# ChantalMP/RaDialog

Measured on AMD Instinct MI355X. Metric: reports_per_sec (448px CXR encode + 160-tok prefill + 256-tok greedy decode), higher is better.
Workload: dtype bf16; 1 GPU; configs[1]: per-GPU batch 1 BioViL-T(ResNet-50)+Q-Former encode 448px, Vicuna-7B prefill T=160, 256-token greedy decode (LoRA r=8 un-merged, hipGraph ; per_gpu_batch=1, global_batch=1, prompt_len=160, parallelism=dp1

## Files before the change

### include/rdx_dec_hooks.h

```cpp
#ifndef RDX_DEC_HOOKS_H
#define RDX_DEC_HOOKS_H
#include "rdx.h"
#ifdef __cplusplus
extern "C" {
#endif

int rdx_xstat16_test(rdx_ctx* ctx, const void* X, const void* norm_w, float eps, const float* W, int M, int N, int epi, int n_valid, void* out,
                     int ldo, int out_packed, int32_t* argmax_host);

int rdx_xrow16_test(rdx_ctx* ctx, const void* X, int x_packed, const float* W, const void* resid, int M, int N, int K, void* out, int ldo);

int rdx_xstat_blk_test(rdx_ctx* ctx, const void* X, const void* norm_w, float eps, const float* W, const void* resid, int M, int N, int epi,
                       int n_valid, void* out, int ldo, int out_packed, void* xp_out, int32_t* argmax_host);

int rdx_xsplit_blk_test(rdx_ctx* ctx, const void* X, const float* W, void* x_resid, const void* norm_w, float eps, int M, int N, float* slab_out,
                        void* xn_out);

int rdx_xstat_blk8_test(rdx_ctx* ctx, const void* X, const void* norm_w, float eps, const float* W, int M, int N, int epi, int n_valid, void* out,
                        int ldo, int out_packed, void* x8_out, float* xscale_out, int32_t* argmax_host);

int rdx_xsplit_blk8_test(rdx_ctx* ctx, const void* X, const float* W, void* x_resid, const void* norm_w, float eps, int M, int N, int K,
                         float* slab_out, void* x8_out, float* xscale_out);

int rdx_rmsnorm_test(rdx_ctx* ctx, void* x, const void* norm_w, float eps, int rows, int H, int layout, int mtiles, const float* slab, int groups, void* out,
                     long long out_bytes, float* xscale, int xscale_n);

int rdx_select_test(rdx_ctx* ctx, void* logits_inout, int B, int vocab, const int32_t* hist, const int32_t* hist_len, const int32_t* n_generated, int ld,
                    const rdx_logits_rules* rules, int eos_id, int32_t* tokens_out);

int rdx_decode_attn_test(rdx_ctx* ctx, int heads, int B, int max_len, int k_perm, int lora_r, float lora_scale, const void* qkv, const void* lbq, const void* lbv,
                         const void* cur_rope, const void* cos_t, const void* sin_t, int max_pos, const int32_t* pos, const int32_t* slot,
                         const uint8_t* key_mask, void* kcache, void* vcache, void* out, long long out_bytes, int out_packed, int out_mt);

int rdx_rope_kv_test(rdx_ctx* ctx, int heads, int B, int T, int max_len, int k_perm, int lora_r, float lora_scale, const void* qkv, const void* lbq,
                     const void* lbv, const void* cos_t, const void* sin_t, int max_pos, const int32_t* pos_ids, int slot0, void* kcache, void* vcache,
                     void* qout);

int rdx_sample_test(rdx_ctx* ctx, void* logits_inout, int B, int vocab, const int32_t* hist, const int32_t* hist_len, const int32_t* n_generated, int ld,
                    const rdx_logits_rules* rules, int eos_id, const rdx_sampling* sampling, int32_t* tokens_out);
int rdx_sample_u24_host(uint64_t seed, uint32_t row, uint32_t draw, uint32_t* out);

#ifdef __cplusplus
}
#endif
#endif
```

### radialog_amd/_lib.py

```python
from __future__ import annotations

import ctypes as C
import os

import torch

HERE = os.path.dirname(os.path.abspath(__file__))
LIB_PATH = os.environ.get("RDX_LIB_PATH") or os.path.join(HERE, "librdx.so")
HOOKS_PATH = os.environ.get("RDX_HOOKS_PATH") or os.path.join(HERE, "librdx_hooks.so")

RDX_DTYPE_F16, RDX_DTYPE_BF16 = 0, 1
RDX_W_GEMM, RDX_W_TENSOR, RDX_W_F32, RDX_W_GEMM_FP8 = 0, 1, 2, 3
RDX_SRC_F32, RDX_SRC_F16, RDX_SRC_BF16 = 0, 1, 2


class RdxLibraryError(RuntimeError):
    pass


class RdxError(RuntimeError):
    pass


class RdxLogitsRules(C.Structure):
# ... 66 lines not shown
    "rdx_quant_test": (C.c_int, [_P, _P, C.c_int, C.c_int, C.c_int, C.c_int, _P, C.c_float, _P, _P]),
    "rdx_gemv_trace": (C.c_int, [_P, C.c_int, C.c_int, _P, C.c_int]),
    "rdx_gemm_test": (C.c_int, [_P, _P, _P, _P, _P, _P, C.c_int, C.c_int, C.c_int, C.c_int, _P, C.c_float, C.c_int]),
    "rdx_kernel_bench": (C.c_int, [_P, C.c_int, C.c_int, C.c_int, C.c_int, C.c_int, C.c_int, C.c_int, C.c_int, C.POINTER(C.c_float), _P, C.c_int]),
    "rdx_conv_test": (C.c_int, [_P, _P, _P, _P, _P, _P, C.c_int, C.c_int, C.c_int, C.c_int, C.c_int, C.c_int, C.c_int, C.c_int, C.c_int, C.POINTER(C.c_float)]),
    "rdx_l2_bench": (C.c_int, [_P, C.c_int, C.c_longlong, C.c_int, C.c_int, C.c_int, C.POINTER(C.c_float)]),
    "rdx_logits_test": (C.c_int, [_P, _P, _P, C.c_int, C.c_int, C.c_int, C.c_int, _P, _P, C.c_int]),
}

TRACE_CHAIN = 7
TRACE_ATTN_OPROJ = 8

ENC_HOOK_SYMBOLS = {
    "rdx_stem_test": (C.c_int, [_P, _P, _P, _P, _P, C.c_int, C.c_int, C.c_int, C.c_int]),
    "rdx_norm_test": (C.c_int, [_P, C.c_int, _P, _P, _P, _P, _P, _P, C.c_int, C.c_int, C.c_longlong, C.c_longlong, C.c_int, C.c_int, C.c_float]),
    "rdx_attn_test": (C.c_int, [_P, _P, _P, _P, _P, _P, C.c_int, C.c_int, C.c_int, C.c_int, C.c_int, C.c_int, _P, C.c_longlong, C.c_int, C.c_int]),
}

_F = C.c_float
DEC_HOOK_SYMBOLS = {
    "rdx_xstat16_test": (C.c_int, [_P, _P, _P, _F, _P, C.c_int, C.c_int, C.c_int, C.c_int, _P, C.c_int, C.c_int, _P]),
    "rdx_xrow16_test": (C.c_int, [_P, _P, C.c_int, _P, _P, C.c_int, C.c_int, C.c_int, _P, C.c_int]),
    "rdx_xstat_blk_test": (C.c_int, [_P, _P, _P, _F, _P, _P, C.c_int, C.c_int, C.c_int, C.c_int, _P, C.c_int, C.c_int, _P, _P]),
    "rdx_xsplit_blk_test": (C.c_int, [_P, _P, _P, _P, _P, _F, C.c_int, C.c_int, _P, _P]),
    "rdx_xstat_blk8_test": (C.c_int, [_P, _P, _P, _F, _P, C.c_int, C.c_int, C.c_int, C.c_int, _P, C.c_int, C.c_int, _P, _P, _P]),
    "rdx_xsplit_blk8_test": (C.c_int, [_P, _P, _P, _P, _P, _F, C.c_int, C.c_int, C.c_int, _P, _P, _P]),
    "rdx_rmsnorm_test": (C.c_int, [_P, _P, _P, _F, C.c_int, C.c_int, C.c_int, C.c_int, _P, C.c_int, _P, C.c_longlong, _P, C.c_int]),
    "rdx_select_test": (C.c_int, [_P, _P, C.c_int, C.c_int, _P, _P, _P, C.c_int, C.POINTER(RdxLogitsRules), C.c_int, _P]),
    "rdx_sample_test": (C.c_int, [_P, _P, C.c_int, C.c_int, _P, _P, _P, C.c_int, C.POINTER(RdxLogitsRules), C.c_int, C.POINTER(RdxSampling), _P]),
    "rdx_sample_u24_host": (C.c_int, [C.c_uint64, C.c_uint32, C.c_uint32, C.POINTER(C.c_uint32)]),
    "rdx_decode_attn_test": (C.c_int, [_P, C.c_int, C.c_int, C.c_int, C.c_int, C.c_int, _F, _P, _P, _P, _P, _P, _P, C.c_int, _P, _P, _P, _P, _P, _P, C.c_longlong,
                                       C.c_int, C.c_int]),
    "rdx_rope_kv_test": (C.c_int, [_P, C.c_int, C.c_int, C.c_int, C.c_int, C.c_int, C.c_int, _F, _P, _P, _P, _P, _P, C.c_int, _P, C.c_int, _P, _P, _P]),
}
ALL_HOOK_SYMBOLS = {**HOOK_SYMBOLS, **ENC_HOOK_SYMBOLS, **DEC_HOOK_SYMBOLS}

_lib = None
_hooks = None


def hooks_enabled() -> bool:
    return os.environ.get("RDX_DEBUG_HOOKS", "0") not in ("", "0")


def _missing_hook(name):
    def raiser(*_a, **_k):
        raise RdxLibraryError(f"{name} is a kernel-test hook of librdx_hooks.so (include/rdx_hooks.h, rdx_enc_hooks.h, rdx_dec_hooks.h), not part of the product library: "
                              "set RDX_DEBUG_HOOKS=1 before radialog_amd is loaded (tests/conftest.py and the tools/ scripts do)")
    return raiser


def load_hooks(lib):
    global _hooks
    if not hooks_enabled():
        for name in ALL_HOOK_SYMBOLS:
            setattr(lib, name, _missing_hook(name))
        return
    src = lib
    if not hasattr(lib, next(iter(HOOK_SYMBOLS))):
        if os.environ.get("RDX_LIB_PATH") and os.path.realpath(LIB_PATH) != os.path.realpath(os.path.join(HERE, "librdx.so")):
            raise RdxLibraryError(f"RDX_DEBUG_HOOKS is set, but RDX_LIB_PATH={LIB_PATH} does not link the hooks in and {HOOKS_PATH} would load a "
                                  "second librdx.so next to it: build the alternative library with api_debug.hip (tools/sanitize_host.sh does)")
        if not os.path.exists(HOOKS_PATH):
            raise RdxLibraryError(f"RDX_DEBUG_HOOKS is set but {HOOKS_PATH} is missing: build it with `python -m radialog_amd.build`")
        try:
            src = C.CDLL(HOOKS_PATH, mode=C.RTLD_GLOBAL)
# ... 65 lines not shown
```

### radialog_amd/csrc/api.hip

```cpp
#include "rdx_ctx.h"

static std::string g_create_err;

int fail(rdx_ctx* c, int code, const char* fmt, ...) {
    char buf[512];
    va_list ap;
    va_start(ap, fmt);
    vsnprintf(buf, sizeof(buf), fmt, ap);
    va_end(ap);
    if (c) c->err = buf; else g_create_err = buf;
    return code;
}

const char* create_error() { return g_create_err.c_str(); }

int dalloc(rdx_ctx* c, void** p, size_t bytes) {
    if (bytes == 0) bytes = 16;
    hipError_t e = hipMalloc(p, bytes);
    if (e != hipSuccess) return fail(c, -3, "hipMalloc(%zu bytes) failed: %s", bytes, hipGetErrorString(e));
    c->allocs.push_back(*p);
    return 0;
}

extern "C" int rdx_create(rdx_ctx** out, int device_id, const rdx_config* cfg) {
// ... 169 lines not shown
}

extern "C" int rdx_finalize_weights(rdx_ctx* c) {
    if (!c) return -1;
    if (c->finalized) return fail(c, -1, "rdx_finalize_weights: already finalized");
    HIPCHK(c, hipSetDevice(c->device));
    const rdx_config& f = c->cfg;
    Resolver R{c};
    if (f.enable_llama) {
        const int H = f.hidden, I = f.inter, r2 = 2 * f.lora_r;
        c->embed = R.t("embed", (int64_t)f.vocab * H);
        c->final_norm = R.t("final_norm", H);
        c->rope_cos = R.t("rope.cos", (int64_t)f.max_pos * 128);
        c->rope_sin = R.t("rope.sin", (int64_t)f.max_pos * 128);
        c->lm_head = R.g("lm_head", f.vocab, H);
        c->img_proj_w = R.g("img_proj.w", H, f.qformer_dim);
        c->img_proj_b = R.f("img_proj.b", H);
        c->ll.resize(f.layers);
        for (int l = 0; l < f.layers; ++l) {
            LlamaLayer& L = c->ll[l];
            L.attn_norm = R.t(S("l%d.attn_norm", l), H);
            L.mlp_norm = R.t(S("l%d.mlp_norm", l), H);
            L.wqkv = R.g(S("l%d.wqkv", l), 3 * H + r2, H);
            L.wo = R.g(S("l%d.wo", l), H, H);
            L.wgu = R.g(S("l%d.wgu", l), 2 * I, H);
            L.wdown = R.g(S("l%d.wdown", l), H, I);
            L.lora_bq = L.lora_bv = nullptr;
            if (f.lora_r) {
                L.lora_bq = R.t(S("l%d.lora_bq", l), (int64_t)H * f.lora_r);
                L.lora_bv = R.t(S("l%d.lora_bv", l), (int64_t)H * f.lora_r);
            }
        }
        if (R.rc) return R.rc;
        c->ld.hidden = H; c->ld.heads = f.heads; c->ld.head_dim = 128; c->ld.qkv_ld = c->ll[0].wqkv.Npad;
        c->ld.lora_r = f.lora_r; c->ld.lora_scale = f.lora_scale; c->ld.max_len = f.max_len; c->ld.max_pos = f.max_pos;
        c->ld.k_perm = (getenv("RDX_KPERM") ? atoi(getenv("RDX_KPERM")) : (f.max_batch * f.heads <= 256)) ? 1 : 0;
        const int B = f.max_batch;
        c->kv_layer_elems = (size_t)B * f.heads * f.max_len * 128;
        ALLOC(c, c->kcache, c->kv_layer_elems * f.layers * 2);
        ALLOC(c, c->vcache, c->kv_layer_elems * f.layers * 2);
        HIPCHK(c, hipMemset(c->kcache, 0, c->kv_layer_elems * f.layers * 2));
        HIPCHK(c, hipMemset(c->vcache, 0, c->kv_layer_elems * f.layers * 2));
        ALLOC(c, c->key_mask, (size_t)B * f.max_len);
        HIPCHK(c, hipMemset(c->key_mask, 0, (size_t)B * f.max_len));
        ALLOC(c, c->d_img_pos, B * sizeof(int)); ALLOC(c, c->d_pos, B * sizeof(int)); ALLOC(c, c->d_slot, B * sizeof(int));
        ALLOC(c, c->d_step, B * sizeof(int)); ALLOC(c, c->d_unf, B * sizeof(int));
        ALLOC(c, c->d_ctr, chain_ctr_ints(f.layers) * sizeof(int)); ALLOC(c, c->d_err, sizeof(int));
        HIPCHK(c, hipMemset(c->d_ctr, 0, chain_ctr_ints(f.layers) * sizeof(int)));
        c->d_cctr = c->d_ctr;
        ALLOC(c, c->d_gran, (size_t)2 * H * 4 + HO_HINT_INTS * sizeof(int)); ALLOC(c, c->d_epoch, sizeof(int));
        HIPCHK(c, hipMemset(c->d_gran, 0, (size_t)2 * H * 4 + HO_HINT_INTS * sizeof(int)));
        HIPCHK(c, hipMemset(c->d_epoch, 0, sizeof(int)));
        c->d_hint = reinterpret_cast<int*>(reinterpret_cast<char*>(c->d_gran) + (size_t)2 * H * 4);
        HIPCHK(c, hipMemset(c->d_err, 0, sizeof(int)));
        ALLOC(c, c->d_cur_rope, (size_t)B * 256 * 2);
        ALLOC(c, c->d_pos_ids, (size_t)B * f.max_len * sizeof(int));
        c->n_vtiles = c->lm_head.Npad / 16;
        ALLOC(c, c->part_val, (size_t)B * c->n_vtiles * sizeof(float));
        ALLOC(c, c->part_idx, (size_t)B * c->n_vtiles * sizeof(int));
        const int Bp = B > 2 ? (B + 31) / 32 * 32 : B;
        ALLOC(c, c->dx, (size_t)B * H * 2); ALLOC(c, c->dxn, (size_t)Bp * H * 2);
        if (B > 2) ALLOC(c, c->kslab, (size_t)4 * Bp * H * sizeof(float));
        ALLOC(c, c->dqkv, (size_t)B * c->ld.qkv_ld * 2);
        ALLOC(c, c->dxs, (size_t)std::max(32, Bp) * sizeof(float));
        ALLOC(c, c->datt, (size_t)Bp * H * 2); ALLOC(c, c->dgu, (size_t)Bp * I * 2);
        ALLOC(c, c->pqe, (size_t)B * 32 * f.qformer_dim * 2); ALLOC(c, c->pimg, (size_t)B * 32 * H * 2);
// ... 60 lines not shown
        if (c->tens.count("v.pool.emb")) {
            const int Cv = f.v_b2v, Pn = v_grid(f) * v_grid(f);
            if (Cv % 32) return fail(c, -1, "ViT pooler needs b2v %% 32 == 0");
            c->pool_emb = R.t("v.pool.emb", (int64_t)2 * Pn * Cv);
            c->pool_ng = R.f("v.pool.norm_g", Cv); c->pool_nb = R.f("v.pool.norm_b", Cv);
            c->v_p1f = R.g("v.proj1f.w", f.v_proj, 2 * Cv); c->v_p1f_b = R.f("v.proj1f.b", f.v_proj);
            for (int i = 0; c->gemm.count(S("v.pool.%d.wqkv", i)); ++i) {
                PoolBlock pb;
                const std::string p = S("v.pool.%d.", i);
                pb.n1_g = R.f(p + "n1_g", Cv); pb.n1_b = R.f(p + "n1_b", Cv); pb.n2_g = R.f(p + "n2_g", Cv); pb.n2_b = R.f(p + "n2_b", Cv);
                pb.wqkv = R.g(p + "wqkv", 3 * Cv, Cv);
                pb.wo = R.g(p + "wo", Cv, Cv); pb.bo = R.f(p + "bo", Cv);
                pb.w1 = R.g(p + "w1", Cv, Cv); pb.b1 = R.f(p + "b1", Cv);
                pb.w2 = R.g(p + "w2", Cv, Cv); pb.b2 = R.f(p + "b2", Cv);
                c->pool.push_back(pb);
            }
        }
    }
    if (R.rc) return R.rc;
    c->finalized = true;
    return 0;
}

extern "C" int rdx_set_option(rdx_ctx* c, const char* name, int value) {
    if (!c || !name) return -1;
    if (!strcmp(name, "flash_min")) { c->flash_min = value; return 0; }
    if (!strcmp(name, "pconv")) { c->trunk_packed = value != 0; return 0; }
    if (!strcmp(name, "prompt_blk")) { c->prompt_blk = value != 0; return 0; }
    if (!strcmp(name, "xs16")) {
        c->xs16 = value != 0;
        if (c->graph) { hipGraphExecDestroy(c->graph); c->graph = nullptr; c->gkey = GraphKey(); }
        return 0;
    }
    return fail(c, -1, "rdx_set_option: unknown option '%s'", name);
}
```

### radialog_amd/csrc/api_debug.hip

```cpp
#include "rdx_ctx.h"
#include "../../include/rdx_hooks.h"
#include "../../include/rdx_enc_hooks.h"

extern "C" int rdx_attn_trace(rdx_ctx* c, int layer, long long* host) {
    if (!c || !c->finalized || c->cur_B <= 0 || !host) return fail(c, -1, "rdx_attn_trace: run a prefill first");
    HIPCHK(c, hipSetDevice(c->device));
    long long* dtr = nullptr;
    HIPCHK(c, hipMalloc(&dtr, 8 * sizeof(long long)));
    HIPCHK(c, hipMemsetAsync(dtr, 0, 8 * sizeof(long long), c->stream));
    DecAttnArgs at = dec_attn_args(c, layer);
    at.trace = dtr;
    launch_decode_attention(c->cfg.dtype, at, c->cur_B, c->stream);
    hipError_t e = hipStreamSynchronize(c->stream);
    if (e == hipSuccess) e = hipMemcpy(host, dtr, 8 * sizeof(long long), hipMemcpyDeviceToHost);
    hipFree(dtr);
    HIPCHK(c, e);
    return 0;
}

extern "C" int rdx_quant_test(rdx_ctx* c, const void* X, int M, int K, int groups, int mode, const void* norm_w, float eps, void* out8, float* scales) {
    if (!c || !X || !out8 || !scales || M <= 0 || K <= 0 || K % 128) return fail(c, -1, "rdx_quant_test: bad arguments (K %% 128 == 0)");
    if (mode == 0 && (groups < 1 || groups > 4)) return fail(c, -1, "rdx_quant_test: 1..4 K groups");
    if (mode == 1 && !norm_w) return fail(c, -1, "rdx_quant_test: mode 1 needs the norm weight");
    HIPCHK(c, hipSetDevice(c->device));
// ... 15 lines not shown
            return fail(c, -1, "rdx_gemv_trace(%d): no room for one more decode step in the KV cache", what);
        const bool fused = c->fuse_attn_oproj && attn_oproj16_supported(c->ld, c->ll[layer].wo.N, c->ll[layer].wo.K, B);
        if (what == 8 && !fused)
            return fail(c, -1, "rdx_gemv_trace(8): the fused attention + o_proj launch is not active in this configuration (batch > 2, RDX_FUSE_AO=0)");
        const int wgs = what == 7 ? H / 16 + ((c->ll[0].wqkv.Npad + 15) / 16 + 3) / 4
                                  : f.heads * B + ((c->ll[layer].wo.N + 15) / 16 + 1) / 2;
        if (wgs > max_tiles) return fail(c, -1, "rdx_gemv_trace(%d): need room for %d workgroups", what, wgs);
        long long* dtr = nullptr;
        const size_t bytes = (size_t)max_tiles * 8 * sizeof(long long);
        HIPCHK(c, hipMalloc(&dtr, bytes));
        HIPCHK(c, hipMemsetAsync(dtr, 0, bytes, c->stream));
        if (what == 7) { c->chain_trace = dtr; c->chain_trace_layer = layer; }
        else { c->ao_trace = dtr; c->ao_trace_layer = layer; }
        const bool chained = decode_step_launch(c, nullptr, nullptr, 0);
        c->chain_trace = nullptr; c->chain_trace_layer = -1;
        c->ao_trace = nullptr; c->ao_trace_layer = -1;
        c->cur_steps = std::max(c->cur_steps + 1, c->cur_max_new);
        hipError_t e = hipStreamSynchronize(c->stream);
        if (e == hipSuccess) e = hipMemcpy(host, dtr, bytes, hipMemcpyDeviceToHost);
        hipFree(dtr);
        HIPCHK(c, e);
        if (what == 7 && !chained) return fail(c, -1, "rdx_gemv_trace(7): the chained down -> QKV launch is not active in this configuration (batch > 2, RDX_CHAIN=0)");
        return 0;
    }
    const LlamaLayer& L = c->ll[layer];
    long long* dtr = nullptr;
    const size_t bytes = (size_t)max_tiles * 8 * sizeof(long long);
    HIPCHK(c, hipMalloc(&dtr, bytes));
    HIPCHK(c, hipMemsetAsync(dtr, 0, bytes, c->stream));
    GemmArgs a = unit_args(c, &L, what == 1 ? UNIT_GATE_UP : what == 2 ? UNIT_QKV : UNIT_DOWN, B);
    if (what != 1 && what != 2) { a.out = c->dqkv; a.resid = nullptr; a.ldr = 0; }
    if ((a.N + 15) / 16 > max_tiles) { hipFree(dtr); return fail(c, -1, "rdx_gemv_trace: need room for %d tiles", (a.N + 15) / 16); }
    a.trace = dtr;
    skinny(c, a, what == 1 ? EPI_SILU_MUL : EPI_NONE);
    hipError_t e = hipStreamSynchronize(c->stream);
    if (e == hipSuccess) e = hipMemcpy(host, dtr, bytes, hipMemcpyDeviceToHost);
    hipFree(dtr);
    HIPCHK(c, e);
    return 0;
}


extern "C" int rdx_kernel_bench(rdx_ctx* c, int rows, int N, int K, int H, int ksize, int stride, int epi, int iters, float* ms_host,
                                long long* trace_host, int trace_wgs) {
    if (!c || !ms_host || iters <= 0 || rows <= 0) return fail(c, -1, "rdx_kernel_bench: bad arguments");
    HIPCHK(c, hipSetDevice(c->device));
    const int Kg = ksize ? ksize * ksize * K : K;
    if (Kg % 32 || N % 16) return fail(c, -1, "rdx_kernel_bench: need K %% 32 == 0 and N %% 16 == 0");
    const int Ho = ksize ? (H + 2 * (ksize / 2) - ksize) / stride + 1 : 0;
    const size_t M = ksize ? (size_t)rows * Ho * Ho : (size_t)rows, Min = ksize ? (size_t)rows * H * H : (size_t)rows;
    char* buf = nullptr;
    const bool kb_wstat = getenv("RDX_KB_WSTAT") && atoi(getenv("RDX_KB_WSTAT")) && !ksize;
    const size_t xb = ((Min + 15) & ~(size_t)15) * K * 2 + 64, wb = (size_t)N * Kg * 2, ob = M * N * 2 + 64, bb = (size_t)N * 4;
    HIPCHK(c, hipMalloc((void**)&buf, xb + wb + 2 * ob + bb));
    HIPCHK(c, hipMemsetAsync(buf, 0, xb + wb + 2 * ob + bb, c->stream));
    GemmW w; w.N = N; w.K = Kg; w.Npad = N; w.w = buf + xb;
    void *out = buf + xb + wb, *res = buf + xb + wb + ob;
    const float* bias = (const float*)(buf + xb + wb + 2 * ob);
    const bool need_res = epi == EPI_RESID || epi == EPI_RESID_RELU;
    hipEvent_t e0, e1;
    HIPCHK(c, hipEventCreate(&e0)); HIPCHK(c, hipEventCreate(&e1));
    struct WsScope { rdx_ctx* c; ~WsScope() { c->ws_ok = false; } } ws_scope{c};
    c->ws_ok = true;
    long long* dtr = nullptr;
    if (trace_host && trace_wgs > 0) { HIPCHK(c, hipMalloc((void**)&dtr, (size_t)trace_wgs * 8 * sizeof(long long))); HIPCHK(c, hipMemset(dtr, 0, (size_t)trace_wgs * 64)); }
    auto once = [&]() {
// ... 92 lines not shown
    HIPCHK(c, hipMalloc((void**)&buf, total + 64));
    HIPCHK(c, hipMemsetAsync(buf, 1, total + 64, c->stream));
    hipEvent_t e0, e1;
    HIPCHK(c, hipEventCreate(&e0)); HIPCHK(c, hipEventCreate(&e1));
    launch_l2_bench(mode, buf, (size_t)bytes_per_wg, shared, 1, wgs, (unsigned*)(buf + total), c->stream);
    HIPCHK(c, hipEventRecord(e0, c->stream));
    launch_l2_bench(mode, buf, (size_t)bytes_per_wg, shared, reps, wgs, (unsigned*)(buf + total), c->stream);
    HIPCHK(c, hipEventRecord(e1, c->stream));
    HIPCHK(c, hipEventSynchronize(e1));
    float ms = 0.f;
    HIPCHK(c, hipEventElapsedTime(&ms, e0, e1));
    hipEventDestroy(e0); hipEventDestroy(e1);
    hipFree(buf);
    HIPCHK(c, hipGetLastError());
    *gbps_host = (float)((double)bytes_per_wg * wgs * reps / (ms * 1e-3) / 1e9);
    return 0;
}

static int fp8_block_for_test(rdx_ctx* c, GemmArgs& a, int epi, char** tmp) {
    *tmp = nullptr;
    if (!(a.W8 && a.wscale) || a.M < xs_min_rows()) return 0;
    GemmArgs t = a; t.norm_w = nullptr;
    if (!xstat32_supported(t, epi)) return 0;
    HIPCHK(c, hipMalloc((void**)tmp, (size_t)32 * a.K + 32 * sizeof(float)));
    float* xs = (float*)(*tmp + (size_t)32 * a.K);
    run_rmsnorm(c, NormArgs{const_cast<void*>(a.X), a.norm_w, *tmp, xs, a.M, a.K, a.eps, ACT_BLK64_E4M3, 0, nullptr, 0});
    a.X = *tmp; a.ldx = a.K; a.xpacked = ACT_BLK64_E4M3; a.xscale = xs; a.xgroups = 1; a.norm_w = nullptr;
    return 0;
}

extern "C" int rdx_gemm_test(rdx_ctx* c, const void* X, const float* W, const float* bias, const void* resid, void* out,
                             int M, int N, int K, int epi, const void* norm_w, float eps, int force) {
    if (!c || !X || !W || !out) return fail(c, -1, "rdx_gemm_test: null argument");
    if (K % 32 || N % 16) return fail(c, -1, "rdx_gemm_test: need K %% 32 == 0 and N %% 16 == 0");
    HIPCHK(c, hipSetDevice(c->device));
    GemmW w;
    w.N = N; w.K = K; w.Npad = N;
    void* wp = nullptr;
    HIPCHK(c, hipMalloc(&wp, (size_t)N * K * 2 + ((force == 4 || (force >= 9 && force <= 11)) ? (size_t)N * K + (size_t)N * 4 : 0)));
    w.w = wp;
    if (force >= 9 && force <= 11) {
        const int G = force == 9 ? 1 : (force == 10 ? 2 : 4);
        if (K % 64 || (norm_w && G != 1)) { hipFree(wp); return fail(c, -1, "rdx_gemm_test: gemm8 needs K %% 64 == 0 (and one K group behind an RMSNorm)"); }
        w.w = nullptr; w.w8 = (char*)wp + (size_t)N * K * 2; w.scale = (float*)((char*)wp + (size_t)N * K * 3);
        launch_pack_weight_fp8(c->cfg.dtype, W, w.w8, w.scale, nullptr, N, K, N, c->stream);
        char* tmp = nullptr;
        if (hipMalloc((void**)&tmp, (size_t)M * K + (size_t)M * 4 * sizeof(float)) != hipSuccess) { hipFree(wp); return fail(c, -2, "rdx_gemm_test: out of device memory"); }
        float* xs = (float*)(tmp + (size_t)M * K);
        if (norm_w) run_rmsnorm(c, NormArgs{const_cast<void*>(X), norm_w, tmp, xs, M, K, eps, ACT_ROWS_E4M3, 0, nullptr, 0});
        else launch_quant_rows(c->cfg.dtype, X, K, tmp, xs, M, K, G, c->stream);
        GemmArgs a = gargs(tmp, K, w, nullptr, out, epi == EPI_SILU_MUL ? N / 2 : N, M);
        a.resid = resid; a.ldr = N; a.xscale = xs; a.xgroups = G;
        int rc = 0;
        if (!gemm8_supported(a, epi)) rc = fail(c, -1, "rdx_gemm_test: shape / epilogue not supported by gemm8");
        else launch_gemm8(c->cfg.dtype, a, epi, c->stream);
        hipError_t se = hipStreamSynchronize(c->stream);
        hipFree(wp); hipFree(tmp);
        if (rc) return rc;
        if (int urc = take_unsupported(c)) return urc;
        HIPCHK(c, se);
        HIPCHK(c, hipGetLastError());
        return 0;
    }
    if (force == 4) {
        if (K % 64) { hipFree(wp); return fail(c, -1, "rdx_gemm_test: fp8 needs K %% 64 == 0"); }
        w.w = nullptr;
        w.w8 = (char*)wp + (size_t)N * K * 2;
        w.scale = (float*)((char*)wp + (size_t)N * K * 3);
        launch_pack_weight_fp8(c->cfg.dtype, W, w.w8, w.scale, nullptr, N, K, N, c->stream);
        force = 1;
    } else
    launch_pack_weight(c->cfg.dtype, W, wp, N, K, N, nullptr, c->stream);
    GemmArgs a = gargs(X, K, w, bias, out, epi == EPI_SILU_MUL ? N / 2 : N, M);
    a.resid = resid; a.ldr = N;
    a.norm_w = norm_w; a.eps = eps;
    void* xn = nullptr;
    bool split8 = false;
    if (force == 6) {
        if (K % 64) { hipFree(wp); return fail(c, -1, "rdx_gemm_test: fp8 needs K %% 64 == 0"); }
        hipFree(wp);
        HIPCHK(c, hipMalloc(&wp, (size_t)N * K * 3 + (size_t)N * 4));
        w.w = nullptr; w.w8 = (char*)wp + (size_t)N * K * 2; w.scale = (float*)((char*)wp + (size_t)N * K * 3);
        launch_pack_weight_fp8(c->cfg.dtype, W, w.w8, w.scale, nullptr, N, K, N, c->stream);
        a = gargs(X, K, w, bias, out, N, M);
        a.resid = resid; a.ldr = N; a.eps = eps;
        split8 = true; force = 5;
    }
    if (force == 5) {
        if (epi != EPI_RESID || !resid || M <= 16 || M > 32) { hipFree(wp); return fail(c, -1, "rdx_gemm_test: force 5 needs epi 3 and 16 < M <= 32"); }
        char* tmp = nullptr;
        const size_t xb = (size_t)32 * K * 2, sb = (size_t)4 * 32 * N * 4;
        if (hipMalloc((void**)&tmp, 2 * xb + sb) != hipSuccess) { hipFree(wp); return fail(c, -2, "rdx_gemm_test: out of device memory"); }
        a.X = tmp; a.xpacked = split8 ? ACT_BLK64 : ACT_BLK32; a.norm_w = nullptr;
        run_rmsnorm(c, NormArgs{const_cast<void*>(X), nullptr, tmp, nullptr, M, K, eps, a.xpacked, 0, nullptr, 0});
        const int kg = xsplit32_groups(a);
        if (!kg) { hipFree(wp); hipFree(tmp); return fail(c, -1, "rdx_gemm_test: shape not supported by xsplit32_k"); }
        launch_xsplit32(c->cfg.dtype, a, (float*)(tmp + 2 * xb), c->stream);
        HIPCHK(c, hipMemcpyAsync(out, resid, (size_t)M * N * 2, hipMemcpyDeviceToDevice, c->stream));
        run_rmsnorm(c, NormArgs{out, nullptr, tmp + xb, nullptr, M, N, eps, ACT_ROWS, 0, (const float*)(tmp + 2 * xb), kg});
        HIPCHK(c, hipStreamSynchronize(c->stream));
        HIPCHK(c, hipGetLastError());
        hipFree(wp); hipFree(tmp);
        return take_unsupported(c);
    }
    if (force == 8) {
        const int mtl = (M + 15) / 16;
        char* tmp = nullptr;
        HIPCHK(c, hipMalloc((void**)&tmp, (size_t)mtl * 16 * K * 2));
// ... 29 lines not shown
            c->dxn = xn;
        }
        skinny(c, a, epi == EPI_RESID_RELU ? EPI_RESID : epi);
        c->dxn = keep;
        hipError_t se = hipStreamSynchronize(c->stream);
        if (blk) hipFree(blk);
        if (int urc = take_unsupported(c)) { hipFree(wp); if (xn) hipFree(xn); return urc; }
        HIPCHK(c, se);
    } else {
        if (a.norm_w) {
            HIPCHK(c, hipMalloc(&xn, (size_t)M * K * 2));
            run_rmsnorm(c, NormArgs{const_cast<void*>(X), norm_w, xn, nullptr, M, K, eps, ACT_ROWS, 0, nullptr, 0});
            a.X = xn; a.norm_w = nullptr;
        }
        ConvGeom cg;
        memset(&cg, 0, sizeof(cg));
        if (force == 3 || (force == 0 && gemm_dma_supported(a))) {
            if (!gemm_dma_supported(a)) { hipFree(wp); if (xn) hipFree(xn); return fail(c, -1, "rdx_gemm_test: shape not supported by gemm_dma_k"); }
            launch_gemm_dma(c->cfg.dtype, a, epi, c->gemm_ws, c->gemm_ws_floats, c->stream);
        } else {
            launch_tiled_gemm(c->cfg.dtype, a, cg, epi, c->stream);
        }
    }
    HIPCHK(c, hipStreamSynchronize(c->stream));
    HIPCHK(c, hipGetLastError());
    hipFree(wp);
    if (xn) hipFree(xn);
    return take_unsupported(c);
}

extern "C" int rdx_logits_test(rdx_ctx* c, const void* X, const float* W, int M, int N, int n_valid, int K, void* out_logits,
                               int32_t* argmax_host, int fp8) {
    if (!c || !X || !W || !out_logits || !argmax_host) return fail(c, -1, "rdx_logits_test: null argument");
    if (K % 32 || N % 16 || M > 32 || n_valid > N || (fp8 && K % 64)) return fail(c, -1, "rdx_logits_test: bad shape");
    HIPCHK(c, hipSetDevice(c->device));
    GemmW w;
    w.N = N; w.K = K; w.Npad = N;
    const int nt = N / 16;
    char* wp = nullptr;
    const size_t wb = (size_t)N * K * 2, qb = fp8 ? (size_t)N * K + (size_t)N * 4 : 0, pb = (size_t)M * nt * 4;
    HIPCHK(c, hipMalloc((void**)&wp, wb + qb + 2 * pb + (size_t)M * K * 2));
    w.w = wp;
    if (fp8) {
        w.w = nullptr; w.w8 = wp + wb; w.scale = (float*)(wp + wb + (size_t)N * K);
        launch_pack_weight_fp8(c->cfg.dtype, W, w.w8, w.scale, nullptr, N, K, N, c->stream);
    } else {
        launch_pack_weight(c->cfg.dtype, W, wp, N, K, N, nullptr, c->stream);
    }
    GemmArgs a = gargs(X, K, w, nullptr, out_logits, N, M);
    a.n_valid = n_valid;
    a.part_val = (float*)(wp + wb + qb); a.part_idx = (int*)(wp + wb + qb + pb);
    char* blk = nullptr;
    int brc = fp8_block_for_test(c, a, EPI_LOGITS, &blk);
    if (brc) { hipFree(wp); return brc; }
    skinny(c, a, EPI_LOGITS);
    std::vector<float> pv((size_t)M * nt);
    std::vector<int> pi((size_t)M * nt);
    hipError_t se = hipStreamSynchronize(c->stream);
    if (blk) hipFree(blk);
    if (int urc = take_unsupported(c)) { hipFree(wp); return urc; }
    HIPCHK(c, se);
    HIPCHK(c, hipGetLastError());
    HIPCHK(c, hipMemcpy(pv.data(), a.part_val, pb, hipMemcpyDeviceToHost));
    HIPCHK(c, hipMemcpy(pi.data(), a.part_idx, pb, hipMemcpyDeviceToHost));
    hipFree(wp);
    for (int m = 0; m < M; ++m) {
        float bv = -INFINITY; int bi = 0x7fffffff;
        for (int t = 0; t < nt; ++t) {
            const float v = pv[(size_t)m * nt + t]; const int ix = pi[(size_t)m * nt + t];
            if (v > bv || (v == bv && ix < bi)) { bv = v; bi = ix; }
        }
        argmax_host[m] = bi;
    }
    return 0;
}


extern "C" int rdx_stem_test(rdx_ctx* c, const float* image, const float* W, const float* bias, void* out, int B, int S, int stem, int path) {
    if (!c || !image || !W || !bias || !out || B <= 0 || S < 16 || S % 4) return fail(c, -1, "rdx_stem_test: bad arguments (S %% 4 == 0, S >= 16)");
    if (path < 0 || path > 2) return fail(c, -1, "rdx_stem_test: path 0 (fused, row-major), 1 (fused, packed) or 2 (conv_gemm + maxpool_k)");
    if (path < 2 && !stem_pool_supported(stem)) return fail(c, -1, "rdx_stem_test: stem_pool_k has no instantiation for %d channels", stem);
    if (path == 2 && stem % 16) return fail(c, -1, "rdx_stem_test: conv_gemm needs stem %% 16 == 0");
    if (path == 1 && !c->zero16) return fail(c, -1, "rdx_stem_test: no zero line for the packed layout");
    HIPCHK(c, hipSetDevice(c->device));
// ... 122 lines not shown
```

### radialog_amd/csrc/api_dec_hooks.hip

```cpp
#include <cmath>

#include "rdx_ctx.h"
#include "philox.h"
#include "../../include/rdx_dec_hooks.h"

namespace {

struct DevBufs {
    std::vector<void*> p;
    ~DevBufs() { for (void* q : p) hipFree(q); }
    void* get(size_t bytes) {
        void* q = nullptr;
        if (hipMalloc(&q, bytes ? bytes : 16) != hipSuccess) return nullptr;
        p.push_back(q);
        return q;
    }
};

int reduce_partials(rdx_ctx* c, const GemmArgs& a, int32_t* argmax_host) {
    const int nt = (a.N + 15) / 16;
    std::vector<float> pv((size_t)a.M * nt);
    std::vector<int> pi((size_t)a.M * nt);
    HIPCHK(c, hipMemcpy(pv.data(), a.part_val, pv.size() * 4, hipMemcpyDeviceToHost));
    HIPCHK(c, hipMemcpy(pi.data(), a.part_idx, pi.size() * 4, hipMemcpyDeviceToHost));
// ... 286 lines not shown
    return finish(c);
}

extern "C" int rdx_sample_test(rdx_ctx* c, void* logits_inout, int B, int vocab, const int32_t* hist, const int32_t* hist_len, const int32_t* n_generated, int ld,
                               const rdx_logits_rules* rules, int eos_id, const rdx_sampling* sm, int32_t* tokens_out) {
    if (!c || !logits_inout || !n_generated || !sm || !tokens_out || B <= 0) return fail(c, -1, "rdx_sample_test: bad arguments");
    const rdx_logits_rules r = rules ? *rules : rdx_logits_rules{1.0f, 0, 0};
    const bool ruled = r.repetition_penalty != 1.0f || r.no_repeat_ngram_size != 0 || r.min_new_tokens != 0;
    if (!(r.repetition_penalty > 0.f) || r.no_repeat_ngram_size < 0 || r.min_new_tokens < 0) return fail(c, -1, "rdx_sample_test: bad rules");
    if (ruled && (!hist || !hist_len || ld <= 0)) return fail(c, -1, "rdx_sample_test: rules need a history");
    if (!(sm->temperature > 0.f) || !std::isfinite(sm->temperature) || sm->top_k < 0 || !(sm->top_p > 0.f) || !(sm->top_p <= 1.0f))
        return fail(c, -1, "rdx_sample_test: bad sampling parameters");
    if (!sample_step_supported(vocab) || (ruled && !select_step_supported(vocab))) return fail(c, -1, "rdx_sample_test: a row of vocab %d does not fit the LDS of sample_step_k", vocab);
    HIPCHK(c, hipSetDevice(c->device));
    if (!c->d_seed) ALLOC(c, c->d_seed, sizeof(unsigned long long));
    const unsigned long long seed = sm->seed;
    HIPCHK(c, hipMemcpyAsync(c->d_seed, &seed, sizeof(seed), hipMemcpyHostToDevice, c->stream));
    SelectArgs a;
    a.logits = logits_inout; a.step_stride = 0; a.n_gen = n_generated;
    a.penalty = r.repetition_penalty; a.ngram = r.no_repeat_ngram_size; a.min_new = r.min_new_tokens; a.sel_out = tokens_out;
    StepTail t = {};
    t.vocab = vocab; t.eos_id = eos_id;
    if (ruled) { t.hist = const_cast<int32_t*>(hist); t.hist_len = const_cast<int32_t*>(hist_len); t.hist_ld = ld; }
    const SampleArgs sp = {sm->temperature, sm->top_k, sm->top_p, c->d_seed};
    launch_sample_step(c->cfg.dtype, a, sp, t, B, c->stream);
    return finish(c);
}

extern "C" int rdx_sample_u24_host(uint64_t seed, uint32_t row, uint32_t draw, uint32_t* out) {
    if (!out) return -1;
    *out = sample_u24(seed, row, draw);
    return 0;
}
```

### radialog_amd/csrc/api_dispatch.hip

```cpp
#include "rdx_ctx.h"

GemmArgs gargs(const void* X, int ldx, const GemmW& W, const float* bias, void* out, int ldo, int M) {
    GemmArgs a;
    memset(&a, 0, sizeof(a));
    a.X = X; a.ldx = ldx; a.W = W.w; a.bias = bias; a.out = out; a.ldo = ldo;
    a.M = M; a.N = W.N; a.K = W.K; a.n_valid = W.N;
    a.W8 = W.w8; a.wscale = W.scale;
    return a;
}

DecAttnArgs dec_attn_args(rdx_ctx* c, int layer) {
    const LlamaLayer& L = c->ll[layer];
    DecAttnArgs at;
    at.d = c->ld; at.qkv = c->dqkv; at.lbq = L.lora_bq; at.lbv = L.lora_bv; at.cos_t = c->rope_cos; at.sin_t = c->rope_sin;
    at.pos = c->d_pos; at.slot_b = c->d_slot; at.key_mask = c->key_mask; at.cur_rope = c->d_cur_rope;
    at.kcache = kv_ptr(c, c->kcache, layer); at.vcache = kv_ptr(c, c->vcache, layer); at.out = c->datt;
    return at;
}

AttnArgs prefill_attn_args(rdx_ctx* c, int B, int T, int keep, int layer) {
    const rdx_config& f = c->cfg;
    const int H = f.hidden;
    AttnArgs at;
    memset(&at, 0, sizeof(at));
    at.Q = c->pq; at.q_bs = (long)T * H; at.q_ts = H; at.q_hs = 128;
    at.K = kv_ptr(c, c->kcache, layer); at.V = kv_ptr(c, c->vcache, layer);
    at.k_bs = at.v_bs = (long)f.heads * f.max_len * 128; at.k_ts = at.v_ts = 128; at.k_hs = at.v_hs = (long)f.max_len * 128;
    at.O = c->patt; at.o_bs = (long)T * H; at.o_ts = H; at.o_hs = 128;
    at.B = B; at.H = f.heads; at.Tq = T; at.Tk = keep + T; at.causal = 1; at.k_perm = c->ld.k_perm; at.key_mask = c->key_mask; at.km_bs = f.max_len;
    at.flash_min = c->flash_min;
    return at;
}

GemmArgs unit_args(rdx_ctx* c, const LlamaLayer* L, DecUnit u, int B) {
    const rdx_config& f = c->cfg;
    const int H = f.hidden;
    GemmArgs a;
    switch (u) {
    case UNIT_QKV: a = gargs(c->dx, H, L->wqkv, nullptr, c->dqkv, c->ld.qkv_ld, B); a.N = L->wqkv.Npad; a.norm_w = L->attn_norm; break;
    case UNIT_O: a = gargs(c->datt, H, L->wo, nullptr, c->dx, H, B); a.resid = c->dx; a.ldr = H; break;
    case UNIT_GATE_UP: a = gargs(c->dx, H, L->wgu, nullptr, c->dgu, f.inter, B); a.norm_w = L->mlp_norm; break;
    case UNIT_DOWN: a = gargs(c->dgu, f.inter, L->wdown, nullptr, c->dx, H, B); a.resid = c->dx; a.ldr = H; break;
    default:
        a = gargs(c->dx, H, c->lm_head, nullptr, nullptr, f.vocab, B);
        a.N = c->lm_head.Npad; a.n_valid = f.vocab; a.norm_w = c->final_norm; a.part_val = c->part_val; a.part_idx = c->part_idx;
    }
    if (a.norm_w) a.eps = f.rms_eps;
    return a;
}

GemmArgs xs16_unit(rdx_ctx* c, const LlamaLayer* L, DecUnit u, int B) {
    GemmArgs a = unit_args(c, L, u, B);
    if (u == UNIT_GATE_UP) a.out_packed = ACT_BLK32;
    if (u == UNIT_O || u == UNIT_DOWN) a.xpacked = ACT_BLK32;
    return a;
}

GemmArgs blk_unit(rdx_ctx* c, const LlamaLayer* L, DecUnit u, int B) {
    GemmArgs a = unit_args(c, L, u, B);
    a.xpacked = ACT_TILES32; a.mtiles = (B + 15) / 16; a.out_packed = u == UNIT_GATE_UP ? ACT_TILES32 : ACT_ROWS;
    return a;
}

GemmArgs blk8_unit(rdx_ctx* c, const LlamaLayer* L, DecUnit u, int B) {
    GemmArgs a = unit_args(c, L, u, B);
    a.xpacked = (u == UNIT_O || u == UNIT_DOWN) ? ACT_BLK64 : ACT_BLK64_E4M3; a.mtiles = (B + 15) / 16; a.out_packed = u == UNIT_GATE_UP ? ACT_BLK64 : ACT_ROWS;
    a.xscale = c->dxs; a.xgroups = 1;
    return a;
}

GemmArgs ksplit_args(GemmArgs a) {
    a.xpacked = (a.W8 && a.wscale) ? ACT_BLK64 : ACT_BLK32;
    return a;
}

GemmArgs prenormed(rdx_ctx* c, GemmArgs a) {
    a.X = c->dxn; a.ldx = a.K; a.norm_w = nullptr;
    return a;
}

void run_rmsnorm(rdx_ctx* c, const NormArgs& n) {
    if (launch_rmsnorm(c->cfg.dtype, n, c->stream)) return;
    char buf[200];
// ... 10 lines not shown
}

DecFamily decode_family(rdx_ctx* c, int B) {
    if (B > 32) return !blk64_ok(c, B) ? DEC_UNSUPPORTED : blk64_fp8(c) ? DEC_BLK8 : DEC_BLK;
    if (c->chain_mlp && c->fuse_attn_oproj && chain_supported(c->ld, c->cfg.inter, B) && attn_oproj16_supported(c->ld, c->cfg.hidden, c->cfg.hidden, B))
        return DEC_CHAINED;
    return xs16_ok(c, B) ? DEC_XS16 : DEC_GENERIC;
}

GemmArgs skinny_prenorm(rdx_ctx* c, GemmArgs a, int epi) {
    if (!a.norm_w) return a;
    const bool xs = xstat32_supported(prenormed(c, a), epi);
    if (skinny_fits_lds(a.M, a.K) && !(a.M >= xs_min_rows() && c->kslab && xs)) return a;
    if (xs && a.W8 && a.wscale) {
        a.xpacked = ACT_BLK64_E4M3; a.xscale = c->dxs; a.xgroups = 1;
    } else if (xs) {
        a.xpacked = ACT_BLK32;
    }
    return norm_in_front(c, a);
}

void skinny(rdx_ctx* c, GemmArgs a, int epi) {
    a = skinny_prenorm(c, a, epi);
    if (!a.W && a.W8) {
        const bool gemv8 = skinny_fits_lds(a.M, a.K) && a.K % 64 == 0 && a.M < xs_min_rows();
        const bool xs8 = a.xpacked == ACT_BLK64_E4M3 && xstat32_supported(a, epi);
        if (!gemv8 && !xs8) {
            char buf[200];
            snprintf(buf, sizeof(buf), "fp8 weights: no kernel for a %d x %d x %d projection at this batch (batch <= 2: M K <= 16 Ki; batch 3-32: K = 4096)", a.M, a.N, a.K);
            c->unsupported = buf;
            return;
        }
    }
    launch_skinny_gemm(c->cfg.dtype, a, epi, c->stream);
}

int take_unsupported(rdx_ctx* c) {
    if (c->unsupported.empty()) return 0;
    const int rc = fail(c, -8, "%s", c->unsupported.c_str());
    c->unsupported.clear();
    return rc;
}

bool down_split_ok(rdx_ctx* c, const LlamaLayer& L, int B) {
    if (B < xs_min_rows() || !c->kslab) return false;
    if (!xstat32_supported(prenormed(c, unit_args(c, &L, UNIT_GATE_UP, B)), EPI_SILU_MUL)) return false;
    return xsplit32_groups(ksplit_args(unit_args(c, &L, UNIT_DOWN, B))) > 0;
}

void launch_ksplit(rdx_ctx* c, const GemmArgs& a) {
    launch_xsplit32(c->cfg.dtype, a, c->kslab, c->stream);
    c->pend_groups = xsplit32_groups(a);
}

void launch_down(rdx_ctx* c, const LlamaLayer& L, int B, bool split) {
    const GemmArgs a = unit_args(c, &L, UNIT_DOWN, B);
    if (split) launch_ksplit(c, ksplit_args(a));
    else skinny(c, a, EPI_RESID);
}

bool blk64_fp8(rdx_ctx* c) { return !c->ll.empty() && fp8_weights(c->ll[0].wqkv); }

bool blk64_ok(rdx_ctx* c, int B) {
    if (B <= 32 || B > RDX_MAX_ROWS || c->ll.empty() || c->cfg.hidden != 4096) return false;
    const LlamaLayer* L = &c->ll[0];
    if (blk64_fp8(c)) {
// ... 49 lines not shown
```

### radialog_amd/csrc/api_inspect.hip

```cpp
#include "rdx_ctx.h"

extern "C" int rdx_kv_read(rdx_ctx* c, int layer, int which, void* dst) {
    if (!c || !c->finalized || !c->cfg.enable_llama) return fail(c, -1, "rdx_kv_read: no llama state");
    if (layer < 0 || layer >= c->cfg.layers || !dst) return fail(c, -1, "rdx_kv_read: bad arguments");
    if (which) HIPCHK(c, hipMemcpyAsync(dst, kv_ptr(c, c->vcache, layer), c->kv_layer_elems * 2, hipMemcpyDeviceToDevice, c->stream));
    else launch_k_unperm(kv_ptr(c, c->kcache, layer), dst, c->kv_layer_elems / ((size_t)c->cfg.max_len * 128), c->cfg.max_len, c->ld.k_perm, c->stream);
    return 0;
}

extern "C" int rdx_hidden_read(rdx_ctx* c, void* dst) {
    if (!c || !c->finalized || !c->cfg.enable_llama || c->cur_B <= 0) return fail(c, -1, "rdx_hidden_read: no llama state");
    HIPCHK(c, hipMemcpyAsync(dst, c->datt, (size_t)c->cur_B * c->cfg.hidden * 2, hipMemcpyDeviceToDevice, c->stream));
    return 0;
}

extern "C" int rdx_time(rdx_ctx* c, int what, int iters, float* ms_host) {
    if (!c || !c->finalized || !c->cfg.enable_llama || c->cur_B <= 0) return fail(c, -1, "rdx_time: run a prefill first");
    if (!ms_host || iters <= 0) return fail(c, -1, "rdx_time: bad arguments");
    HIPCHK(c, hipSetDevice(c->device));
    const rdx_config& f = c->cfg;
    const int dt = f.dtype, B = c->cur_B;
    const bool same_layer = what >= 10;
    if (same_layer) what -= 10;
    const DecFamily fam = decode_family(c, B);
// ... 41 lines not shown
        HIPCHK(c, hipEventRecord(e0, c->stream));
        for (int i = 0; i < iters; ++i) HIPCHK(c, hipGraphLaunch(c->graph, c->stream));
        HIPCHK(c, hipEventRecord(e1, c->stream));
        launches = iters;
        c->cur_steps = std::max(c->cur_steps, c->cur_max_new);
    } else {
        if (!proj && what != 6) { hipEventDestroy(e0); hipEventDestroy(e1); return fail(c, -1, "rdx_time: unknown unit %d", what); }
        const DecUnit u = what == 1 ? UNIT_GATE_UP : what == 2 ? UNIT_QKV : what == 3 ? UNIT_O : what == 4 ? UNIT_DOWN : UNIT_LM_HEAD;
        const int epi = what == 1 ? EPI_SILU_MUL : what == 5 ? EPI_LOGITS : EPI_NONE;
        const bool resid_unit = u == UNIT_O || u == UNIT_DOWN;
        x16 = proj && fam == DEC_XS16;
        GemmArgs pn;
        bool hoisted = false;
        if (proj && !x16 && !resid_unit) { pn = skinny_prenorm(c, unit_args(c, &c->ll[0], u, B), epi); hoisted = !pn.norm_w; }
        HIPCHK(c, hipEventRecord(e0, c->stream));
        for (int i = 0; i < iters; ++i) {
            for (int l = 0; l < (what == 5 ? 1 : f.layers); ++l, ++launches) {
                const int li = same_layer ? 0 : l;
                const LlamaLayer* L = &c->ll[li];
                if (what == 6) {
                    launch_decode_attention(dt, dec_attn_args(c, li), B, c->stream);
                } else if (x16) {
                    GemmArgs a = xs16_unit(c, L, u, B);
                    if (resid_unit) { a.out = c->dqkv; launch_xrow16(dt, a, c->stream); }
                    else launch_xstat16(dt, a, epi, c->stream);
                } else if (resid_unit) {
                    GemmArgs a = unit_args(c, L, u, B);
                    a.out = c->dqkv; a.resid = nullptr; a.ldr = 0;
                    const bool split = u == UNIT_O ? B >= xs_min_rows() && c->kslab && xsplit32_groups(ksplit_args(a)) : down_split_ok(c, *L, B);
                    if (split) launch_xsplit32(dt, ksplit_args(a), c->kslab, c->stream);
                    else skinny(c, a, EPI_NONE);
                } else {
                    GemmArgs a = unit_args(c, L, u, B);
                    if (hoisted) { a = prenormed(c, a); a.xpacked = pn.xpacked; a.xscale = pn.xscale; a.xgroups = pn.xgroups; }
                    launch_skinny_gemm(dt, a, epi, c->stream);
                }
            }
        }
        HIPCHK(c, hipEventRecord(e1, c->stream));
    }
    HIPCHK(c, hipEventSynchronize(e1));
    float ms = 0.f;
    HIPCHK(c, hipEventElapsedTime(&ms, e0, e1));
    hipEventDestroy(e0); hipEventDestroy(e1);
    *ms_host = ms / (float)launches;
    return x16 ? take_unsupported(c) : 0;
}
```

### radialog_amd/csrc/api_llama.hip

```cpp
#include <cmath>

#include "rdx_ctx.h"

static int ensure_prefill_ws(rdx_ctx* c, size_t rows) {
    rows = (rows + 15) & ~(size_t)15;
    if (rows <= c->prefill_rows) return 0;
    const rdx_config& f = c->cfg;
    HIPCHK(c, hipStreamSynchronize(c->stream));
    c->prefill_rows = 0;
    dfree(c, c->px); dfree(c, c->pxn); dfree(c, c->pqkv); dfree(c, c->pq); dfree(c, c->patt); dfree(c, c->pgu); dfree(c, c->pxq); dfree(c, c->pxs); dfree(c, c->pslab);
    if (fp8_weights(c->ll[0].wqkv)) {
        ALLOC(c, c->pxq, rows * (size_t)std::max(f.hidden, f.inter));
        ALLOC(c, c->pxs, rows * 4 * sizeof(float));
    }
    ALLOC(c, c->px, rows * f.hidden * 2); ALLOC(c, c->pxn, rows * f.hidden * 2);
    ALLOC(c, c->pslab, (size_t)4 * std::min<size_t>(rows, 192) * f.hidden * sizeof(float));
    ALLOC(c, c->pqkv, rows * c->ld.qkv_ld * 2); ALLOC(c, c->pq, rows * f.hidden * 2);
    ALLOC(c, c->patt, rows * f.hidden * 2); ALLOC(c, c->pgu, rows * f.inter * 2);
    c->prefill_rows = rows;
    return 0;
}

static const char* const k_need_blk = "more than 32 decoder rows need hidden 4096 / inter 11008 (the row-block family)";

static void lm_head_and_greedy(rdx_ctx* c, const void* x, int B, void* logits, const int* out_step, long step_stride,
                               int advance) {
    const rdx_config& f = c->cfg;
    if ((c->rules_on || c->sampling.do_sample) && !logits) { logits = c->rule_logits; out_step = nullptr; }
    auto lm = [&](GemmArgs a) { a.X = x; a.out = logits; a.out_step = out_step; a.out_step_stride = step_stride; return a; };
    switch (decode_family(c, B)) {
    case DEC_UNSUPPORTED: c->unsupported = k_need_blk; return;
    case DEC_BLK: launch_xstat_blk(f.dtype, norm_in_front(c, lm(blk_unit(c, nullptr, UNIT_LM_HEAD, B))), EPI_LOGITS, c->stream); break;
    case DEC_BLK8: launch_xstat_blk8(f.dtype, norm_in_front(c, lm(blk8_unit(c, nullptr, UNIT_LM_HEAD, B))), EPI_LOGITS, c->stream); break;
    case DEC_XS16:
        if (x == c->dx) { launch_xstat16(f.dtype, lm(xs16_unit(c, nullptr, UNIT_LM_HEAD, B)), EPI_LOGITS, c->stream); break; }
        [[fallthrough]];
    default: skinny(c, lm(unit_args(c, nullptr, UNIT_LM_HEAD, B)), EPI_LOGITS);
    }
    StepTail t = {};
    t.eos_id = c->cur_eos; t.pad_id = c->cur_pad; t.max_new = c->cur_max_new; t.out_tokens = c->cur_tokens; t.unfinished = c->d_unf;
    t.pos = advance ? c->d_pos : nullptr; t.slot_b = advance ? c->d_slot : nullptr; t.step_b = c->d_step;
    t.embed = c->embed; t.vocab = f.vocab; t.x_next = c->dx; t.H = f.hidden; t.pos_ro = c->d_pos; t.cos_t = c->rope_cos; t.sin_t = c->rope_sin;
    t.cur_rope = c->d_cur_rope;
    t.ctr_zero = c->chain_mlp ? c->d_ctr : nullptr;
    t.n_zero = (int)chain_ctr_ints(f.layers);
    t.epoch = c->d_epoch;
    if (!c->rules_on && !c->sampling.do_sample) { launch_greedy_step(f.dtype, c->part_val, c->part_idx, c->n_vtiles, B, t, c->stream); return; }
    if (c->rules_on) { t.hist = c->d_hist; t.hist_len = c->d_hist_len; t.hist_ld = f.max_len; }
    SelectArgs sa;
    sa.logits = logits; sa.step_stride = out_step ? step_stride : 0; sa.n_gen = c->d_step;
    sa.penalty = c->rules.repetition_penalty; sa.ngram = c->rules.no_repeat_ngram_size; sa.min_new = c->rules.min_new_tokens; sa.sel_out = nullptr;
    if (!c->sampling.do_sample) { launch_select_step(f.dtype, sa, t, B, c->stream); return; }
    const SampleArgs sp = {c->sampling.temperature, c->sampling.top_k, c->sampling.top_p, c->d_seed};
    launch_sample_step(f.dtype, sa, sp, t, B, c->stream);
}

static const rdx_sampling k_sampling_off = {0, 1.0f, 0, 1.0f, 0};

extern "C" int rdx_set_sampling(rdx_ctx* c, const rdx_sampling* sm) {
    if (!c) return -1;
    if (!sm || !sm->do_sample) { c->sampling = k_sampling_off; return 0; }
    const rdx_sampling v = *sm;
    if (!(v.temperature > 0.f) || !std::isfinite(v.temperature)) return fail(c, -1, "rdx_set_sampling: temperature must be a finite float > 0 (1.0 = off)");
    if (v.top_k < 0) return fail(c, -1, "rdx_set_sampling: top_k %d is negative (0 = off)", v.top_k);
    if (!(v.top_p > 0.f) || !(v.top_p <= 1.0f)) return fail(c, -1, "rdx_set_sampling: top_p must be in (0, 1] (1.0 = off)");
    if (!c->finalized || !c->cfg.enable_llama) return fail(c, -1, "rdx_set_sampling: llama weights not finalized");
    const rdx_config& f = c->cfg;
    if (!sample_step_supported(f.vocab)) return fail(c, -1, "rdx_set_sampling: a row of vocab %d does not fit the LDS of sample_step_k", f.vocab);
    HIPCHK(c, hipSetDevice(c->device));
    if (!c->rule_logits) ALLOC(c, c->rule_logits, (size_t)f.max_batch * f.vocab * 2);
// ... 235 lines not shown
    const int kg = (B >= xs_min_rows() && c->kslab) ? xsplit32_groups(ap) : 0;
    at.out_packed = kg > 0 ? ap.xpacked : ACT_ROWS;
    launch_decode_attention(dt, at, B, c->stream);
    if (kg) launch_ksplit(c, ap);
    else skinny(c, ao, EPI_RESID);
}

static void step_generic(rdx_ctx* c, int B) {
    for (int l = 0; l < c->cfg.layers; ++l) {
        const LlamaLayer& L = c->ll[l];
        skinny(c, unit_args(c, &L, UNIT_QKV, B), EPI_NONE);
        attn_oproj(c, l, B);
        const bool split = down_split_ok(c, L, B);
        GemmArgs gu = unit_args(c, &L, UNIT_GATE_UP, B);
        gu.out_packed = split ? ksplit_args(unit_args(c, &L, UNIT_DOWN, B)).xpacked : ACT_ROWS;
        skinny(c, gu, EPI_SILU_MUL);
        launch_down(c, L, B, split);
    }
}

static void step_chained(rdx_ctx* c, int B, std::vector<hipEvent_t>* evs) {
    const rdx_config& f = c->cfg;
    hipStream_t s = c->stream;
    ChainArgs ca;
    memset(&ca, 0, sizeof(ca));
    ca.hidden = f.hidden; ca.inter = f.inter; ca.qkv_n = c->ll[0].wqkv.Npad; ca.qkv_ld = c->ld.qkv_ld; ca.B = B; ca.eps = f.rms_eps;
    ca.dx = c->dx; ca.dqkv = c->dqkv; ca.dgu = c->dgu; ca.ctr = c->d_cctr; ca.err = c->d_err; ca.naps = c->chain_naps;
    const LlamaLayer& L0 = c->ll[0];
    ca.w8 = (L0.wqkv.w8 && L0.wdown.w8 && f.hidden % 64 == 0 && f.inter % 64 == 0) ? 1 : 0;
    auto mark = [&] { if (evs) { hipEvent_t e; hipEventCreate(&e); hipEventRecord(e, s); evs->push_back(e); } };
    skinny(c, unit_args(c, &L0, UNIT_QKV, B), EPI_NONE);
    for (int l = 0; l < f.layers; ++l) {
        attn_oproj(c, l, B);
        skinny(c, unit_args(c, &c->ll[l], UNIT_GATE_UP, B), EPI_SILU_MUL);
        mark();
        ca.layer = l;
        {
            const LlamaLayer& L = c->ll[l];
            const LlamaLayer* Ln = l + 1 < f.layers ? &c->ll[l + 1] : nullptr;
            ca.wdown = L.wdown.w; ca.wdown8 = L.wdown.w8; ca.sdown = L.wdown.scale;
            ca.wqkv = Ln ? Ln->wqkv.w : nullptr; ca.wqkv8 = Ln ? Ln->wqkv.w8 : nullptr; ca.sqkv = Ln ? Ln->wqkv.scale : nullptr;
            ca.attn_norm = Ln ? Ln->attn_norm : nullptr;
        }
        ca.trace = l == c->chain_trace_layer ? c->chain_trace : nullptr;
        launch_decode_chain(f.dtype, ca, l + 1 < f.layers, s);
        mark();
    }
}

bool decode_step_launch(rdx_ctx* c, void* logits, const int* out_step, long step_stride, std::vector<hipEvent_t>* evs) {
    const int B = c->cur_B;
    const DecFamily fam = decode_family(c, B);
    switch (fam) {
    case DEC_UNSUPPORTED: c->unsupported = k_need_blk; return false;
    case DEC_BLK: step_blk(c, B); break;
    case DEC_BLK8: step_blk8(c, B); break;
    case DEC_XS16: step_xs16(c, B); break;
    case DEC_CHAINED: step_chained(c, B, evs); break;
    case DEC_GENERIC: step_generic(c, B); break;
    }
    lm_head_and_greedy(c, c->dx, B, logits, out_step, step_stride, 1);
    return fam == DEC_CHAINED;
}

extern "C" int rdx_decode_step(rdx_ctx* c, void* logits) {
    if (!c) return -1;
    if (!c->finalized || c->cur_B <= 0) return fail(c, -1, "rdx_decode_step: no prefill has run");
    if (c->cur_steps >= c->cur_max_new)
        return fail(c, -1, "rdx_decode_step: all %d tokens of this prompt (max_new) have been generated; run a new prefill", c->cur_max_new);
    if (c->cur_T + c->cur_steps > c->cfg.max_len || c->cur_T + c->cur_steps > c->cfg.max_pos)
        return fail(c, -1, "rdx_decode_step: KV cache full (%d prompt + %d generated slots of %d)", c->cur_T, c->cur_steps, c->cfg.max_len);
    if (int rrc = rules_need_prefill(c, "rdx_decode_step")) return rrc;
    HIPCHK(c, hipSetDevice(c->device));
    decode_step_launch(c, logits, nullptr, 0);
    ++c->cur_steps;
// ... 254 lines not shown
```

### radialog_amd/csrc/chain.hip

```cpp
#include "rdx_common.h"
#include "rdx_kernels.h"
#include "attn_body.h"
#include "handoff.h"
#include "skinny_body.h"

namespace rdx {

constexpr int CH_WAVES = 16;
constexpr int CH_THREADS = CH_WAVES * 64;
constexpr int CH_MAXM = 2;

struct ChainGemm {
    const void* X; int ldx;
    const void* resid; int ldr;
    void* out; int ldo;
    int M, N;
    const void* norm_w; float eps;
    const float* wscale;
};

template <typename WaitFn> struct ChainLate { ChainGemm a; WaitFn wait; long long* trace; };

template <typename T, int EPI, bool NORM, int SUB, int XL, typename WaitFn, int U = 4, bool RESID_EARLY = false, bool W8 = false, typename Late>
__device__ __forceinline__ ChainLate<WaitFn> chain_tile(const void* Wb, const int K, const int wg, const int ntiles, unsigned char* smem, Late late) {
    typedef typename Vec8<T>::type V8;
    constexpr int WPS = CH_WAVES / SUB;
    float* red = reinterpret_cast<float*>(smem);
    float* ssq = red + CH_WAVES * 256;
    float* rstd_s = ssq + CH_WAVES * CH_MAXM;
    T* xs = reinterpret_cast<T*>(rstd_s + 16);

    const int lane = threadIdx.x & 63, wa = __builtin_amdgcn_readfirstlane(threadIdx.x >> 6);
    const int sub = wa / WPS, w = wa - sub * WPS;
    const int tile = wg * SUB + sub;
    const int tile_c = min(tile, ntiles - 1);
    const int r = lane & 15, g = lane >> 4;
    const int KC = W8 ? (K >> 6) : (K >> 5);
    const int c0 = (KC * w) / WPS, c1 = (KC * (w + 1)) / WPS;
    const u4* wbase = reinterpret_cast<const u4*>(Wb) + (size_t)tile_c * KC * 64 + lane;
    const int clast = min(max(c1 - 1, c0), KC - 1);
    const long long t_entry = (long long)__builtin_amdgcn_s_memrealtime();

    u4 wa_[U], wb_[U];
#pragma unroll
    for (int u = 0; u < U; ++u) wa_[u] = ldg16_nt(wbase + (size_t)min(c0 + u, clast) * 64);
#pragma unroll
    for (int u = 0; u < U; ++u) wb_[u] = ldg16_nt(wbase + (size_t)min(c0 + U + u, clast) * 64);
    __builtin_amdgcn_sched_barrier(0);
    const ChainLate<WaitFn> lt = late();
    const ChainGemm& a = lt.a;
    const WaitFn& wait_inputs = lt.wait;
    long long* const trace = lt.trace;
    const T* X = reinterpret_cast<const T*>(a.X);
    long long* trc = (trace && threadIdx.x == 0) ? trace : nullptr;
#define CH_T(i) do { if (trc) trc[i] = (long long)__builtin_amdgcn_s_memrealtime(); } while (0)
    if (trc) trc[0] = t_entry;
    if (trace) {
        if (threadIdx.x < 64) asm volatile("s_waitcnt vmcnt(%0)" :: "n"(2 * U - 1) : "memory");
        CH_T(5);
    }

    constexpr int QPT_E = EPI == EPI_SILU_MUL ? 2 : 4;
    unsigned long long rs8_early = 0ull;
    if (RESID_EARLY && EPI == EPI_RESID && (int)threadIdx.x < SUB * a.M * QPT_E) {
        const int so = threadIdx.x / (a.M * QPT_E), rem = threadIdx.x - so * (a.M * QPT_E);
        const int m = rem / QPT_E, q = rem - m * QPT_E;
        const int n = (wg * SUB + so) * 16 + q * 4;
        if (wg * SUB + so < ntiles && n < a.N) rs8_early = ld8_agent(reinterpret_cast<const T*>(a.resid) + (size_t)m * a.ldr + n);
    }

    wait_inputs();
    if (!WaitFn::TAGGED) CH_T(3);

    const int K4 = K >> 2, total4 = a.M * K4;
    unsigned long long xr[XL];
    if constexpr (WaitFn::TAGGED) {
        wait_inputs.template sweep<XL>(xr, a.X, a.ldx, K4, total4, CH_THREADS);
        if (trace) __syncthreads();
        CH_T(3);
    } else {
#pragma unroll
        for (int i = 0; i < XL; ++i) {
            const int c = threadIdx.x + i * CH_THREADS;
            xr[i] = 0ull;
            if (c < total4) { const int m = c / K4, k4 = c - m * K4; xr[i] = ld8_agent(X + (size_t)m * a.ldx + (size_t)k4 * 4); }
        }
    }
    if (NORM) {
        float ss[CH_MAXM];
#pragma unroll
        for (int m = 0; m < CH_MAXM; ++m) ss[m] = 0.f;
// ... 13 lines not shown
            if (lane == 0) ssq[wa * CH_MAXM + m] = t;
        }
        __syncthreads();
        if (threadIdx.x < CH_MAXM) {
            float t = 0.f;
#pragma unroll
            for (int i = 0; i < CH_WAVES; ++i) t += ssq[i * CH_MAXM + threadIdx.x];
            rstd_s[threadIdx.x] = rsqrtf(t / (float)K + a.eps);
        }
        __syncthreads();
    }
    {
        const T* NW = reinterpret_cast<const T*>(a.norm_w);
#pragma unroll
        for (int i = 0; i < XL; ++i) {
            const int c = threadIdx.x + i * CH_THREADS;
            if (c < total4) {
                const int m = c / K4, k4 = c - m * K4;
                unsigned long long v = xr[i];
                if (NORM) {
                    const float rs = rstd_s[m];
                    const unsigned long long nw = *reinterpret_cast<const unsigned long long*>(NW + (size_t)k4 * 4);
                    v = 0ull;
#pragma unroll
                    for (int j = 0; j < 4; ++j) {
                        const float h = rnd<T>(tof<T>(from_bits16<T>((unsigned short)(xr[i] >> (16 * j)))) * rs);
                        const float wv_ = tof<T>(from_bits16<T>((unsigned short)(nw >> (16 * j))));
                        v |= (unsigned long long)bits16<T>(fromf<T>(wv_ * h)) << (16 * j);
                    }
                }
                *reinterpret_cast<unsigned long long*>(xs + (size_t)m * K + (size_t)k4 * 4) = v;
            }
        }
        __syncthreads();
    }

    const T* xrow = xs + (size_t)(r < a.M ? r : 0) * K + g * (W8 ? 16 : 8);
    v4f acc = (v4f){0.f, 0.f, 0.f, 0.f};
    CH_T(6);
    auto consume = [&](const u4 (&wreg)[U], int cb, bool guard) {
#pragma unroll
        for (int u = 0; u < U; ++u) {
            if (!guard || cb + u < c1) {
                if (W8) {
#pragma unroll
                    for (int h = 0; h < 2; ++h) {
                        const u4 wd = dequant8<T>(h ? wreg[u].z : wreg[u].x, h ? wreg[u].w : wreg[u].y);
                        const u4 xv = *reinterpret_cast<const u4*>(xrow + (size_t)(cb + u) * 64 + h * 8);
                        acc = mfma16(as_vec8<T>(wd), as_vec8<T>(xv), acc);
                    }
                } else {
                    const u4 xv = *reinterpret_cast<const u4*>(xrow + (size_t)(cb + u) * 32);
                    acc = mfma16(as_vec8<T>(wreg[u]), as_vec8<T>(xv), acc);
                }
            }
        }
    };
    auto consume1 = [&](const u4& wv, int c) {
        if (W8) {
#pragma unroll
            for (int h = 0; h < 2; ++h) {
                const u4 wd = dequant8<T>(h ? wv.z : wv.x, h ? wv.w : wv.y);
                const u4 xv = *reinterpret_cast<const u4*>(xrow + (size_t)c * 64 + h * 8);
                acc = mfma16(as_vec8<T>(wd), as_vec8<T>(xv), acc);
            }
        } else {
            const u4 xv = *reinterpret_cast<const u4*>(xrow + (size_t)c * 32);
            acc = mfma16(as_vec8<T>(wv), as_vec8<T>(xv), acc);
        }
    };
    int cb = c0;
    for (; cb + 2 * U < c1; cb += 2 * U) {
#pragma unroll
        for (int u = 0; u < 2 * U; ++u) {
            u4& wr = u < U ? wa_[u] : wb_[u - U];
            consume1(wr, cb + u);
            wr = ldg16_nt(wbase + (size_t)min(cb + 2 * U + u, clast) * 64);
            __builtin_amdgcn_sched_barrier(0);
        }
    }
    consume(wa_, cb, true);
    consume(wb_, cb + U, true);
    CH_T(1);
    *reinterpret_cast<float4*>(&red[wa * 256 + r * 16 + g * 4]) = make_float4(acc[0], acc[1], acc[2], acc[3]);
    __syncthreads();

    T* out = reinterpret_cast<T*>(a.out);
    constexpr int QPT = EPI == EPI_SILU_MUL ? 2 : 4;
    const int items = SUB * a.M * QPT;
    if ((int)threadIdx.x < items) {
        const int so = threadIdx.x / (a.M * QPT), rem = threadIdx.x - so * (a.M * QPT);
        const int m = rem / QPT, q = rem - m * QPT;
        const int t_o = wg * SUB + so;
        const int n = t_o * 16 + q * 4;
        const bool ok = (t_o < ntiles) && (n < a.N);
        float v[4];
#pragma unroll
        for (int j = 0; j < 4; ++j) {
            v[j] = 0.f;
#pragma unroll
            for (int i = 0; i < WPS; ++i) v[j] += red[(so * WPS + i) * 256 + m * 16 + q * 4 + j];
            if (W8) v[j] *= a.wscale[t_o * 16 + q * 4 + j];
        }
        unsigned long long pk = 0ull;
        if (EPI == EPI_NONE) {
#pragma unroll
            for (int j = 0; j < 4; ++j) pk |= (unsigned long long)bits16<T>(fromf<T>(v[j])) << (16 * j);
            if (ok) st8_agent(out + (size_t)m * a.ldo + n, pk);
        } else if (EPI == EPI_RESID) {
            if (ok) {
                const unsigned long long rs8 = RESID_EARLY ? rs8_early : ld8_agent(reinterpret_cast<const T*>(a.resid) + (size_t)m * a.ldr + n);
#pragma unroll
                for (int j = 0; j < 4; ++j) {
                    const float rsd = tof<T>(from_bits16<T>((unsigned short)(rs8 >> (16 * j))));
                    pk |= (unsigned long long)bits16<T>(fromf<T>(rsd + rnd<T>(v[j]))) << (16 * j);
// ... 8 lines not shown
                for (int i = 0; i < WPS; ++i) u += red[(so * WPS + i) * 256 + m * 16 + 8 + q * 4 + j];
                if (W8) u *= a.wscale[t_o * 16 + 8 + q * 4 + j];
                pk |= (unsigned long long)bits16<T>(fromf<T>(swiglu<T>(v[j], u))) << (16 * j);
            }
            if (ok) st8_agent(out + (size_t)m * a.ldo + t_o * 8 + q * 4, pk);
        }
    }
    CH_T(7);
#undef CH_T
    return lt;
}

template <typename T, bool W8>
__global__ __launch_bounds__(CH_THREADS, 4) void decode_chain_k(const void* wdown, const void* wqkv, int hidden, int inter, int qkv_n, int nwg_down, ChainArgs) {
    extern __shared__ __attribute__((aligned(16))) unsigned char msm[];
    const int H = hidden;
    auto args = [] { return late_kernarg<ChainArgs>(kernarg_offset<6>(decltype(&decode_chain_k<T, W8>){})); };
    if ((int)blockIdx.x < nwg_down) {
        const ChainLate<WaitSharded> lt = chain_tile<T, EPI_RESID, false, 1, 6, WaitSharded, 4, false, W8>(wdown, inter, blockIdx.x, nwg_down, msm, [&] {
            const ChainArgs ca = args();
            int* ctr = ca.ctr + (size_t)ca.layer * HO_CTR_INTS;
            return ChainLate<WaitSharded>{ChainGemm{ca.dgu, inter, ca.dx, H, ca.dx, H, ca.B, H, nullptr, 0.f, ca.sdown},
                                          WaitSharded{ctr, 0, ca.err, ca.naps, nullptr}, ca.trace ? ca.trace + (size_t)blockIdx.x * 8 : nullptr};
        });
        publish_sc1(lt.wait.ctr, blockIdx.x);
        if (lt.trace && threadIdx.x == 0) lt.trace[2] = (long long)__builtin_amdgcn_s_memrealtime();
        return;
    }
    chain_tile<T, EPI_NONE, true, 4, 2, WaitSharded, W8 ? 4 : 8, false, W8>(wqkv, H, blockIdx.x - nwg_down, (qkv_n + 15) / 16, msm, [&] {
        const ChainArgs ca = args();
        int* ctr = ca.ctr + (size_t)ca.layer * HO_CTR_INTS;
        return ChainLate<WaitSharded>{ChainGemm{ca.dx, H, nullptr, 0, ca.dqkv, ca.qkv_ld, ca.B, qkv_n, ca.attn_norm, ca.eps, ca.sqkv},
                                      WaitSharded{ctr, nwg_down, ca.err, ca.naps, nullptr}, ca.trace ? ca.trace + (size_t)blockIdx.x * 8 : nullptr};
    });
}

template <typename Kernel> struct AttnOprojLate {
    static constexpr unsigned AT = kernarg_offset<10>(Kernel{}), G = kernarg_offset<11>(Kernel{}), HINT = kernarg_offset<12>(Kernel{}), ERR = kernarg_offset<13>(Kernel{});
    __device__ __forceinline__ DecAttnArgs operator()() const { return late_kernarg<DecAttnArgs>(AT); }
    __device__ __forceinline__ int* hint() const { return late_kernarg<int*>(HINT) + blockIdx.x; }
};
template <typename T, bool W8>
__global__ __launch_bounds__(CH_THREADS, 4) void attn_oproj16_k(const void* wo, const void* qkv, void* kcache, void* vcache, int K, int ntiles, int n_attn,
                                                                 int max_len, int qkv_ld, int k_perm, DecAttnArgs, ChainGemm, int*, int*) {
    extern __shared__ __attribute__((aligned(16))) unsigned char msm[];
    if ((int)blockIdx.x < n_attn) {
        const int heads = K >> 7;
        const int b = blockIdx.x / heads, h = blockIdx.x - b * heads;
        const AttnEarly e = {qkv, kcache, vcache, LlamaDims{K, heads, 128, qkv_ld, 0, 0.f, max_len, 0, k_perm}};
        const AttnOprojLate<decltype(&attn_oproj16_k<T, W8>)> late;
        decode_attention_core<T, CH_WAVES, true, NoWait, true, 0, true, false>(e, late, h, b, reinterpret_cast<float*>(msm), NoWait());
        const DecAttnArgs at = late();
        if (at.trace && threadIdx.x == 0) {
            asm volatile("s_waitcnt vmcnt(0)" ::: "memory");
            at.trace[(size_t)blockIdx.x * 8 + 6] = (long long)__builtin_amdgcn_s_memrealtime();
        }
    } else {
        chain_tile<T, EPI_RESID, false, 2, 2, WaitTagged, W8 ? 4 : 8, true, W8>(wo, K, blockIdx.x - n_attn, ntiles, msm, [&] {
            typedef AttnOprojLate<decltype(&attn_oproj16_k<T, W8>)> L;
            const DecAttnArgs at = late_kernarg<DecAttnArgs>(L::AT);
            const ChainGemm g = late_kernarg<ChainGemm>(L::G);
            int* hint = late_kernarg<int*>(L::HINT);
            int* err = late_kernarg<int*>(L::ERR);
            return ChainLate<WaitTagged>{g, WaitTagged{hint, n_attn, at.epoch, at.layers, at.layer, err}, at.trace ? at.trace + (size_t)blockIdx.x * 8 : nullptr};
        });
    }
// ... 3 lines not shown
    const int ntiles = (N + 15) / 16;
    return B <= CH_MAXM && d.head_dim == 128 && K == d.heads * 128 && K == d.hidden && K % 32 == 0 && N % 4 == 0 && (size_t)B * K <= 8192 &&
           d.heads * B + (ntiles + 1) / 2 <= 256;
}

void launch_attn_oproj16(int dtype, const DecAttnArgs& a, const GemmArgs& ga, int B, int* hint, int* err, hipStream_t s) {
    const int n_attn = a.d.heads * B, ntiles = (ga.N + 15) / 16;
    const bool w8 = ga.W8 && ga.wscale && ga.K % 64 == 0;
    ChainGemm g = {ga.X, ga.ldx, ga.resid, ga.ldr, ga.out, ga.ldo, ga.M, ga.N, nullptr, 0.f, ga.wscale};
    const size_t sm_gemm = (size_t)(CH_WAVES * 256 + CH_WAVES * CH_MAXM + 16) * 4 + (size_t)B * ga.K * 2;
    const size_t sm_att = decode_attention_smem_floats(CH_WAVES, a.d.max_len) * sizeof(float);
    const size_t smem = sm_gemm > sm_att ? sm_gemm : sm_att;
    dim3 grid(n_attn + (ntiles + 1) / 2), block(CH_THREADS);
    RDX_DISPATCH_T(dtype, T, {
        if (w8) hipLaunchKernelGGL((attn_oproj16_k<T, true>), grid, block, smem, s, ga.W8, a.qkv, a.kcache, a.vcache, ga.K, ntiles, n_attn, a.d.max_len, a.d.qkv_ld,
                                   a.d.k_perm, a, g, hint, err);
        else hipLaunchKernelGGL((attn_oproj16_k<T, false>), grid, block, smem, s, ga.W, a.qkv, a.kcache, a.vcache, ga.K, ntiles, n_attn, a.d.max_len, a.d.qkv_ld,
                                a.d.k_perm, a, g, hint, err);
    });
}

bool chain_supported(const LlamaDims& d, int inter, int B) {
    if (B > CH_MAXM || d.head_dim != 128 || d.hidden % 32 || inter % 32 || d.hidden % 16) return false;
    const size_t stage = (size_t)B * (inter > d.hidden ? inter : d.hidden) * 2;
    return stage <= 48 * 1024 && inter % 4 == 0 && (size_t)B * d.hidden <= 8192 && (size_t)B * inter <= 24576;
}

size_t chain_ctr_ints(int layers) { return (size_t)layers * HO_CTR_INTS; }

void launch_decode_chain(int dtype, ChainArgs ca, bool with_next_qkv, hipStream_t s) {
    const int nwg_down = ca.hidden / 16;
    const int nwg_qkv = with_next_qkv ? ((ca.qkv_n + 15) / 16 + 3) / 4 : 0;
    const int kmax = ca.inter > ca.hidden ? ca.inter : ca.hidden;
    const size_t sm_gemm = (size_t)(CH_WAVES * 256 + CH_WAVES * CH_MAXM + 16) * 4 + (size_t)ca.B * kmax * 2;
    const size_t smem = sm_gemm > (size_t)84 * 1024 ? sm_gemm : (size_t)84 * 1024;
    dim3 grid(nwg_down + nwg_qkv), block(CH_THREADS);
    RDX_DISPATCH_T(dtype, T, {
        static DevOnce attr_set;
        if (attr_set.first()) {
            hipFuncSetAttribute((const void*)decode_chain_k<T, false>, hipFuncAttributeMaxDynamicSharedMemorySize, 100 * 1024);
            hipFuncSetAttribute((const void*)decode_chain_k<T, true>, hipFuncAttributeMaxDynamicSharedMemorySize, 100 * 1024);
        }
        if (ca.w8) hipLaunchKernelGGL((decode_chain_k<T, true>), grid, block, smem, s, ca.wdown8, ca.wqkv8, ca.hidden, ca.inter, ca.qkv_n, nwg_down, ca);
        else hipLaunchKernelGGL((decode_chain_k<T, false>), grid, block, smem, s, ca.wdown, ca.wqkv, ca.hidden, ca.inter, ca.qkv_n, nwg_down, ca);
    });
}

}
```

### radialog_amd/csrc/gemm.hip

```cpp
#include "rdx_common.h"
#include "rdx_kernels.h"
#include "skinny_body.h"

namespace rdx {

template <typename T>
__global__ void pack_weight_k(const float* __restrict__ src, T* __restrict__ dst, int N, int K, int Npad,
                              const int* __restrict__ rowmap) {
    const int K8 = K >> 3;
    const size_t idx = (size_t)blockIdx.x * blockDim.x + threadIdx.x;
    if (idx >= (size_t)Npad * K8) return;
    const int i = (int)(idx / K8), k8 = (int)(idx % K8);
    int srow = rowmap ? rowmap[i] : i;
    if (srow >= N) srow = -1;
    typename Vec8<T>::type v;
    if (srow >= 0) {
        const float4* s = reinterpret_cast<const float4*>(src + (size_t)srow * K + (size_t)k8 * 8);
        float4 a = s[0], b = s[1];
        v[0] = fromf<T>(a.x); v[1] = fromf<T>(a.y); v[2] = fromf<T>(a.z); v[3] = fromf<T>(a.w);
        v[4] = fromf<T>(b.x); v[5] = fromf<T>(b.y); v[6] = fromf<T>(b.z); v[7] = fromf<T>(b.w);
    } else {
#pragma unroll
        for (int j = 0; j < 8; ++j) v[j] = fromf<T>(0.f);
    }
// ... 29 lines not shown
        for (int j = 0; j < 16; ++j) w[j] = real ? src[(size_t)i * K + (size_t)q * 16 + j] * inv : 0.f;
        unsigned d[4];
#pragma unroll
        for (int j = 0; j < 4; ++j) {
            int v = 0;
            v = __builtin_amdgcn_cvt_pk_fp8_f32(w[4 * j], w[4 * j + 1], v, false);
            v = __builtin_amdgcn_cvt_pk_fp8_f32(w[4 * j + 2], w[4 * j + 3], v, true);
            d[j] = (unsigned)v;
        }
        const int kc = q >> 2, g = q & 3;
        reinterpret_cast<u4*>(dst8)[((size_t)nt * KC8 + kc) * 64 + (g * 16 + r)] = (u4){d[0], d[1], d[2], d[3]};
        if (dst)
#pragma unroll
        for (int h = 0; h < 2; ++h) {
            typename Vec8<T>::type v;
#pragma unroll
            for (int j = 0; j < 2; ++j) {
                const auto f0 = __builtin_amdgcn_cvt_pk_f32_fp8((int)d[2 * h + j], false);
                const auto f1 = __builtin_amdgcn_cvt_pk_f32_fp8((int)d[2 * h + j], true);
                v[4 * j] = fromf<T>(f0[0] * sc); v[4 * j + 1] = fromf<T>(f0[1] * sc);
                v[4 * j + 2] = fromf<T>(f1[0] * sc); v[4 * j + 3] = fromf<T>(f1[1] * sc);
            }
            const int k0 = q * 16 + h * 8;
            reinterpret_cast<u4*>(dst)[((size_t)nt * KC + (k0 >> 5)) * 64 + (((k0 & 31) >> 3) * 16 + r)] = as_u4<T>(v);
        }
    }
}

void launch_pack_weight_fp8(int dtype, const float* src, void* dst8, float* scale, void* dst, int N, int K, int Npad, hipStream_t s) {
    RDX_DISPATCH_T(dtype, T, hipLaunchKernelGGL((pack_weight_fp8_k<T>), dim3(Npad), dim3(256), 0, s, src, (unsigned char*)dst8,
                                                scale, (T*)dst, N, K, Npad));
}

template <typename T, int MT, int EPI, bool NORM, int WAVES, bool XLDS, bool W8 = false>
__global__ __launch_bounds__(WAVES * 64, WAVES == 4 ? 8 : 1) void skinny_gemm_k(const void* Wb, const void* X, int K, int N, GemmArgs) {
    extern __shared__ __attribute__((aligned(16))) unsigned char dyn_smem[];
    skinny_tile<T, MT, EPI, NORM, WAVES, XLDS, NoWait, false, W8>(Wb, K, blockIdx.x, (N + 15) / 16, dyn_smem, NoWait(), [&] {
        constexpr unsigned off = kernarg_offset<4>(decltype(&skinny_gemm_k<T, MT, EPI, NORM, WAVES, XLDS, W8>){});
        GemmArgs a = late_kernarg<GemmArgs>(off);
        a.X = X; a.K = K; a.N = N;
        return a;
    });
}

template <typename T, int MT, bool NORM, int WAVES, bool XLDS, bool W8 = false>
static void launch_skinny_epi(const GemmArgs& a, int epi, hipStream_t s) {
    const int nt = (a.N + 15) / 16;
    dim3 grid(nt), block(WAVES * 64);
    const size_t dyn = XLDS ? (size_t)a.M * a.K * 2 : 0;
#define RDX_SK(E) hipLaunchKernelGGL((skinny_gemm_k<T, MT, E, NORM, WAVES, XLDS, W8>), grid, block, dyn, s, W8 ? a.W8 : a.W, a.X, a.K, a.N, a)
    switch (epi) {
        case EPI_NONE: RDX_SK(EPI_NONE); break;
        case EPI_RELU: RDX_SK(EPI_RELU); break;
        case EPI_GELU: RDX_SK(EPI_GELU); break;
        case EPI_RESID: RDX_SK(EPI_RESID); break;
        case EPI_SILU_MUL: RDX_SK(EPI_SILU_MUL); break;
        case EPI_LOGITS: RDX_SK(EPI_LOGITS); break;
        default: break;
    }
#undef RDX_SK
}

bool skinny_fits_lds(int M, int K) { return M <= 16 && (size_t)M * K * 2 <= 32 * 1024; }

template <typename T>
static void launch_skinny_T(const GemmArgs& a, int epi, hipStream_t s) {
    const bool norm = a.norm_w != nullptr;
    constexpr int WV = 8;
    constexpr bool wide = true;
    const bool w8 = a.W8 && a.wscale && skinny_fits_lds(a.M, a.K) && a.K % 64 == 0;
    if (wide && skinny_fits_lds(a.M, a.K) && (a.N + 15) / 16 <= 256 && a.K >= 4096) {
        if (w8) { if (norm) launch_skinny_epi<T, 1, true, 16, true, true>(a, epi, s); else launch_skinny_epi<T, 1, false, 16, true, true>(a, epi, s); return; }
        if (norm) launch_skinny_epi<T, 1, true, 16, true>(a, epi, s); else launch_skinny_epi<T, 1, false, 16, true>(a, epi, s);
        return;
    }
    constexpr bool smallwg = true;
    if (smallwg && skinny_fits_lds(a.M, a.K) && (a.N + 15) / 16 > 512 && (size_t)a.M * a.K * 2 <= 16 * 1024) {
        if (w8) { if (norm) launch_skinny_epi<T, 1, true, 4, true, true>(a, epi, s); else launch_skinny_epi<T, 1, false, 4, true, true>(a, epi, s); return; }
        if (norm) launch_skinny_epi<T, 1, true, 4, true>(a, epi, s); else launch_skinny_epi<T, 1, false, 4, true>(a, epi, s);
        return;
    }
    if (skinny_fits_lds(a.M, a.K)) {
        if (w8) { if (norm) launch_skinny_epi<T, 1, true, WV, true, true>(a, epi, s); else launch_skinny_epi<T, 1, false, WV, true, true>(a, epi, s); return; }
        if (norm) launch_skinny_epi<T, 1, true, WV, true>(a, epi, s); else launch_skinny_epi<T, 1, false, WV, true>(a, epi, s);
    } else if (a.M <= 16) {
        launch_skinny_epi<T, 1, false, WV, false>(a, epi, s);
    } else {
        launch_skinny_epi<T, 2, false, WV, false>(a, epi, s);
    }
}

void launch_skinny_gemm(int dtype, const GemmArgs& a, int epi, hipStream_t s) {
    if (xstat32_supported(a, epi) && (!(a.W8 && a.wscale) || (a.xpacked == ACT_BLK64_E4M3 && a.xscale))) { launch_xstat32(dtype, a, epi, s); return; }
    RDX_DISPATCH_T(dtype, T, launch_skinny_T<T>(a, epi, s));
}

constexpr int TG_BM = 128, TG_BN = 128;

template <typename T>
__device__ __forceinline__ u4 gather_a(const T* X, const GemmArgs& a, const ConvGeom& cg, bool rowok, size_t rowbase,
                                       int ih0, int iw0, int k) {
    if (!rowok) return (u4){0u, 0u, 0u, 0u};
    if (cg.mode == 0) return ldg16(X + rowbase + k);
    const int kpos = k / cg.Cin, c0 = k - kpos * cg.Cin;
    const int kh = kpos / cg.KW, kw = kpos - kh * cg.KW;
    const int ih = ih0 + kh, iw = iw0 + kw;
    if (ih < 0 || ih >= cg.Hin || iw < 0 || iw >= cg.Win) return (u4){0u, 0u, 0u, 0u};
    return ldg16(X + rowbase + ((size_t)ih * cg.Win + iw) * cg.Cin + c0);
}

template <typename T, int EPI>
__global__ __launch_bounds__(256) void tiled_gemm_k(GemmArgs a, ConvGeom cg) {
    typedef typename Vec8<T>::type V8;
    __shared__ __attribute__((aligned(16))) u4 Xs[2][8][64];

    const int MB = (a.M + TG_BM - 1) / TG_BM, NB = (a.N + TG_BN - 1) / TG_BN;
    const int nwg = MB * NB;
    int tile;
    {
        const int id = blockIdx.x, xcd = id & 7, q = nwg >> 3, rr = nwg & 7;
        tile = (xcd < rr ? xcd * (q + 1) : rr * (q + 1) + (xcd - rr) * q) + (id >> 3);
    }
    const int bn = tile / MB, bm = tile - bn * MB;
    const int M0 = bm * TG_BM, N0 = bn * TG_BN;

    const int t = threadIdx.x, lane = t & 63, w = __builtin_amdgcn_readfirstlane(t >> 6);
// ... 156 lines not shown
```

### radialog_amd/csrc/rdx_common.h

```cpp
#pragma once
#include <hip/hip_runtime.h>
#include <stdint.h>
#include <math.h>
#include "rdx_kernels.h"

namespace rdx {

typedef _Float16 f16;
typedef __bf16 bf16;
typedef float v4f __attribute__((ext_vector_type(4)));
typedef unsigned int u4 __attribute__((ext_vector_type(4)));
typedef unsigned int u2 __attribute__((ext_vector_type(2)));
typedef _Float16 v8h __attribute__((ext_vector_type(8)));
typedef __bf16 v8b __attribute__((ext_vector_type(8)));

enum DType { DT_F16 = 0, DT_BF16 = 1 };

template <typename T> __device__ __forceinline__ float tof(T x) { return (float)x; }
template <typename T> __device__ __forceinline__ T fromf(float x) { return (T)x; }
template <typename T> __device__ __forceinline__ float rnd(float x) { return (float)((T)x); }

template <typename T> struct Vec8;
template <> struct Vec8<f16> { typedef v8h type; };
template <> struct Vec8<bf16> { typedef v8b type; };
// ... 17 lines not shown
    return r;
}
template <int I, typename... A> constexpr unsigned kernarg_offset(void (*)(A...)) { return kernarg_offset_of<I, A...>(); }
template <typename A> __device__ __forceinline__ A late_kernarg(unsigned offset) {
    typedef __attribute__((address_space(4))) const unsigned char kbyte;
    typedef __attribute__((address_space(4))) const A kA;
    kA* p = (kA*)((kbyte*)__builtin_amdgcn_kernarg_segment_ptr() + offset);
    asm volatile("" : "+s"(p) :: "memory");
    A a;
    __builtin_memcpy(&a, p, sizeof(A));
    return a;
}
__device__ __forceinline__ u4 ldg16(const void* p) { return *(const g_u4*)p; }
__device__ __forceinline__ u4 ldg16_nt(const void* p) { return __builtin_nontemporal_load((const g_u4*)p); }
__device__ __forceinline__ void stg16(void* p, u4 v) { *(g_u4*)p = v; }

template <typename T> __device__ __forceinline__ u4 dequant8(unsigned lo, unsigned hi);
template <> __device__ __forceinline__ u4 dequant8<bf16>(unsigned lo, unsigned hi) {
    const auto a = __builtin_amdgcn_cvt_pk_f32_fp8((int)lo, false), b = __builtin_amdgcn_cvt_pk_f32_fp8((int)lo, true);
    const auto c = __builtin_amdgcn_cvt_pk_f32_fp8((int)hi, false), d = __builtin_amdgcn_cvt_pk_f32_fp8((int)hi, true);
    const float a0 = a[0], a1 = a[1], b0 = b[0], b1 = b[1], c0 = c[0], c1 = c[1], d0 = d[0], d1 = d[1];
    return (u4){__builtin_amdgcn_perm(__builtin_bit_cast(unsigned, a1), __builtin_bit_cast(unsigned, a0), 0x07060302u),
                __builtin_amdgcn_perm(__builtin_bit_cast(unsigned, b1), __builtin_bit_cast(unsigned, b0), 0x07060302u),
                __builtin_amdgcn_perm(__builtin_bit_cast(unsigned, c1), __builtin_bit_cast(unsigned, c0), 0x07060302u),
                __builtin_amdgcn_perm(__builtin_bit_cast(unsigned, d1), __builtin_bit_cast(unsigned, d0), 0x07060302u)};
}
template <> __device__ __forceinline__ u4 dequant8<f16>(unsigned lo, unsigned hi) {
    const auto a = __builtin_amdgcn_cvt_pk_f32_fp8((int)lo, false), b = __builtin_amdgcn_cvt_pk_f32_fp8((int)lo, true);
    const auto c = __builtin_amdgcn_cvt_pk_f32_fp8((int)hi, false), d = __builtin_amdgcn_cvt_pk_f32_fp8((int)hi, true);
    return (u4){__builtin_bit_cast(unsigned, __builtin_amdgcn_cvt_pkrtz(a[0], a[1])), __builtin_bit_cast(unsigned, __builtin_amdgcn_cvt_pkrtz(b[0], b[1])),
                __builtin_bit_cast(unsigned, __builtin_amdgcn_cvt_pkrtz(c[0], c[1])), __builtin_bit_cast(unsigned, __builtin_amdgcn_cvt_pkrtz(d[0], d[1]))};
}

__device__ __forceinline__ void fp8_scale(float amax, float& sc, float& inv) {
    sc = amax > 0.f ? amax / 448.0f : 1.0f;
    inv = amax > 0.f ? 448.0f / amax : 1.0f;
}
template <typename T> __device__ __forceinline__ u2 quant8(const typename Vec8<T>::type& v, float inv) {
    int lo = 0, hi = 0;
    lo = __builtin_amdgcn_cvt_pk_fp8_f32(tof<T>(v[0]) * inv, tof<T>(v[1]) * inv, lo, false);
    lo = __builtin_amdgcn_cvt_pk_fp8_f32(tof<T>(v[2]) * inv, tof<T>(v[3]) * inv, lo, true);
    hi = __builtin_amdgcn_cvt_pk_fp8_f32(tof<T>(v[4]) * inv, tof<T>(v[5]) * inv, hi, false);
    hi = __builtin_amdgcn_cvt_pk_fp8_f32(tof<T>(v[6]) * inv, tof<T>(v[7]) * inv, hi, true);
    return (u2){(unsigned)lo, (unsigned)hi};
}
template <typename T> __device__ __forceinline__ float amax8(const typename Vec8<T>::type& v) {
    float m = 0.f;
#pragma unroll
    for (int j = 0; j < 8; ++j) m = fmaxf(m, fabsf(tof<T>(v[j])));
    return m;
}
template <int CTRL> __device__ __forceinline__ float dpp_mov(float v) {
    return __builtin_bit_cast(float, __builtin_amdgcn_update_dpp(0, __builtin_bit_cast(int, v), CTRL, 0xF, 0xF, true));
}
constexpr int DPP_XOR1 = 0xB1, DPP_XOR2 = 0x4E, DPP_HALF_MIRROR = 0x141, DPP_MIRROR = 0x140, DPP_ROR8 = 0x128;
__device__ __forceinline__ float row16_sum(float v) {
    v += dpp_mov<DPP_XOR1>(v);
    v += dpp_mov<DPP_XOR2>(v);
    v += dpp_mov<DPP_HALF_MIRROR>(v);
    v += dpp_mov<DPP_MIRROR>(v);
    return v;
}
__device__ __forceinline__ float row16_max(float v) {
    v = fmaxf(v, dpp_mov<DPP_XOR1>(v));
    v = fmaxf(v, dpp_mov<DPP_XOR2>(v));
    v = fmaxf(v, dpp_mov<DPP_HALF_MIRROR>(v));
// ... 82 lines not shown
```

### radialog_amd/csrc/rdx_ctx.h

```cpp
#pragma once
#include <hip/hip_runtime.h>
#include <stdarg.h>
#include <stdio.h>
#include <stdlib.h>
#include <string.h>

#include <algorithm>
#include <map>
#include <string>
#include <vector>

#include "../../include/rdx.h"
#include "rdx_common.h"
#include "rdx_kernels.h"

using namespace rdx;

constexpr int RDX_MAX_ROWS = 128;

struct GemmW { void* w = nullptr; int N = 0, K = 0, Npad = 0; void* w8 = nullptr; float* scale = nullptr; };
struct RawW { void* p = nullptr; int64_t rows = 0, cols = 0; };

struct LlamaLayer {
    const void *attn_norm, *mlp_norm, *lora_bq, *lora_bv;
    GemmW wqkv, wo, wgu, wdown;
};
struct QLayer {
    GemmW s_wqkv, s_wo, c_wq, c_wo, w1, w2;
    const float *s_bqkv, *s_bo, *s_g, *s_b, *c_bq, *c_bo, *c_g, *c_b, *b1, *b2, *f_g, *f_b;
    int cross_idx;
};
struct VBlock {
    GemmW c1, c2, c3, ds;
    const float *b1, *b2, *b3, *bds;
    bool has_ds;
    int planes, stride;
};

struct PoolBlock {
    const float *n1_g, *n1_b, *n2_g, *n2_b, *bo, *b1, *b2;
    GemmW wqkv, wo, w1, w2;
};

struct GraphKey {
    int B = -1, max_new = 0, eos = 0, pad = 0;
    const void* tokens = nullptr; const void* scores = nullptr;
    bool fixed = false;
    rdx_logits_rules rules = {1.0f, 0, 0};
    rdx_sampling sampling = {0, 1.0f, 0, 1.0f, 0};
    bool operator==(const GraphKey& o) const {
        return B == o.B && max_new == o.max_new && eos == o.eos && pad == o.pad && tokens == o.tokens && scores == o.scores && fixed == o.fixed &&
               rules.repetition_penalty == o.rules.repetition_penalty && rules.no_repeat_ngram_size == o.rules.no_repeat_ngram_size &&
               rules.min_new_tokens == o.rules.min_new_tokens && sampling.do_sample == o.sampling.do_sample &&
// ... 11 lines not shown

    std::map<std::string, GemmW> gemm;
    std::map<std::string, RawW> tens;
    std::map<std::string, RawW> f32;

    std::vector<LlamaLayer> ll;
    const void *embed = nullptr, *final_norm = nullptr, *rope_cos = nullptr, *rope_sin = nullptr;
    GemmW lm_head, img_proj_w;
    const float* img_proj_b = nullptr;
    LlamaDims ld;
    void *kcache = nullptr, *vcache = nullptr;
    size_t kv_layer_elems = 0;
    uint8_t* key_mask = nullptr;
    int *d_img_pos = nullptr, *d_pos_ids = nullptr, *d_pos = nullptr, *d_slot = nullptr, *d_step = nullptr, *d_unf = nullptr;
    float* part_val = nullptr; int* part_idx = nullptr; int n_vtiles = 0;
    void *dx = nullptr, *dxn = nullptr, *dqkv = nullptr, *datt = nullptr, *dgu = nullptr;
    float* dxs = nullptr;
    void* pxq = nullptr; float* pxs = nullptr;
    std::string unsupported;
    float* kslab = nullptr;
    int pend_groups = 0;
    void *px = nullptr, *pxn = nullptr, *pqkv = nullptr, *pq = nullptr, *patt = nullptr, *pgu = nullptr, *pqe = nullptr, *pimg = nullptr;
    size_t prefill_rows = 0;
    float* pslab = nullptr;
    int cur_B = 0, cur_T = 0, cur_max_new = 0, cur_eos = -1, cur_pad = 0;
    int cur_steps = 0;
    int32_t* cur_tokens = nullptr;
    hipGraphExec_t graph = nullptr;
    bool fuse_attn_oproj = true;
    bool chain_mlp = true;
    bool xs16 = true;
    bool prompt_blk = true;
    bool blk_down = true;
    int chain_naps = 1;
    long long* chain_trace = nullptr; int chain_trace_layer = -1;
    long long* ao_trace = nullptr; int ao_trace_layer = -1;
    GemmW cls_fc1, cls_fc2; const float *cls_fc1_b = nullptr, *cls_fc2_b = nullptr;
    void *cls_pooled = nullptr, *cls_h = nullptr, *cls_out = nullptr;
    void* zero16 = nullptr;
    void* d_cur_rope = nullptr;
    int* d_cctr = nullptr;
    int *d_ctr = nullptr, *d_err = nullptr;
    void* d_gran = nullptr; int *d_hint = nullptr, *d_epoch = nullptr;
    int flash_min = 512;
    bool pconv_noks = false;
    bool trunk_packed = true;
    bool ws_ok = false;
    float* gemm_ws = nullptr; size_t gemm_ws_floats = 0;
    GraphKey gkey;
    rdx_logits_rules rules = {1.0f, 0, 0};
    bool hist_ready = false;
    bool rules_on = false;
    int *d_hist = nullptr, *d_hist_len = nullptr;
    void* rule_logits = nullptr;
    rdx_sampling sampling = {0, 1.0f, 0, 1.0f, 0};
    unsigned long long* d_seed = nullptr;

    void* bm_logits = nullptr; float* bm_scores = nullptr; float* bm_cand_s = nullptr; int* bm_cand_i = nullptr;
    int *bm_tok = nullptr, *bm_src = nullptr; int32_t* bm_out = nullptr; void* bm_scratch = nullptr;
    size_t bm_scratch_bytes = 0; int bm_rows = 0, bm_new = 0;

    void* tf_ws = nullptr; size_t tf_bytes = 0;

    void* comm = nullptr; int comm_rank = 0, comm_world = 0;

    std::vector<QLayer> ql;
// ... 15 lines not shown
int fail(rdx_ctx* c, int code, const char* fmt, ...);
const char* create_error();

#define HIPCHK(c, call)                                                                         \
    do {                                                                                        \
        hipError_t e_ = (call);                                                                 \
        if (e_ != hipSuccess) return fail((c), -2, "%s failed: %s (%s:%d)", #call, hipGetErrorString(e_), __FILE__, __LINE__); \
    } while (0)

inline size_t esz(const rdx_ctx* c) { (void)c; return 2; }

int dalloc(rdx_ctx* c, void** p, size_t bytes);
#define ALLOC(c, ptr, bytes) do { int rc_ = dalloc((c), (void**)&(ptr), (bytes)); if (rc_) return rc_; } while (0)

template <typename P>
inline void dfree(rdx_ctx* c, P*& p) {
    if (!p) return;
    auto it = std::find(c->allocs.begin(), c->allocs.end(), (void*)p);
    if (it != c->allocs.end()) c->allocs.erase(it);
    hipFree((void*)p);
    p = nullptr;
}

GemmArgs gargs(const void* X, int ldx, const GemmW& W, const float* bias, void* out, int ldo, int M);
GemmArgs skinny_prenorm(rdx_ctx* c, GemmArgs a, int epi);
void skinny(rdx_ctx* c, GemmArgs a, int epi);
void launch_ksplit(rdx_ctx* c, const GemmArgs& a);
enum DecUnit { UNIT_QKV, UNIT_O, UNIT_GATE_UP, UNIT_DOWN, UNIT_LM_HEAD };
enum DecFamily { DEC_UNSUPPORTED, DEC_CHAINED, DEC_GENERIC, DEC_XS16, DEC_BLK, DEC_BLK8 };
DecFamily decode_family(rdx_ctx* c, int B);
DecAttnArgs dec_attn_args(rdx_ctx* c, int layer);
AttnArgs prefill_attn_args(rdx_ctx* c, int B, int T, int keep, int layer);
GemmArgs unit_args(rdx_ctx* c, const LlamaLayer* L, DecUnit u, int B);
GemmArgs xs16_unit(rdx_ctx* c, const LlamaLayer* L, DecUnit u, int B);
GemmArgs blk_unit(rdx_ctx* c, const LlamaLayer* L, DecUnit u, int B);
GemmArgs blk8_unit(rdx_ctx* c, const LlamaLayer* L, DecUnit u, int B);
GemmArgs ksplit_args(GemmArgs a);
GemmArgs prenormed(rdx_ctx* c, GemmArgs a);
GemmArgs norm_in_front(rdx_ctx* c, GemmArgs a);
void run_rmsnorm(rdx_ctx* c, const NormArgs& n);
bool down_split_ok(rdx_ctx* c, const LlamaLayer& L, int B);
void launch_down(rdx_ctx* c, const LlamaLayer& L, int B, bool split);
bool blk64_ok(rdx_ctx* c, int B);
bool blk64_fp8(rdx_ctx* c);
bool xs16_ok(rdx_ctx* c, int B);
void run_gemm(rdx_ctx* c, GemmArgs a, int epi);
void conv_gemm(rdx_ctx* c, const void* X, const GemmW& W, const float* bias, const void* resid, void* out, int B,
               int Hin, int Win, int Cin, int KH, int KW, int stride, int pad, int Hout, int Wout, int epi);
int run_stem_pool(rdx_ctx* c, const void* vin, const GemmW& W, const float* bias, void* out, int B, int S, bool packed);
int v_grid(const rdx_config& f);
inline bool fp8_weights(const GemmW& W) { return W.w8 && W.scale && !W.w; }
int take_unsupported(rdx_ctx* c);

inline void* kv_ptr(rdx_ctx* c, void* base, int layer) { return (char*)base + (size_t)layer * c->kv_layer_elems * 2; }
int prefill_impl(rdx_ctx* c, const int32_t* ids, const int32_t* mask, int B, int T, const float* qformer_embs, int keep,
                 int max_new, int eos_id, int pad_id, int32_t* out_tokens, void* logits);
bool decode_step_launch(rdx_ctx* c, void* logits, const int* out_step, long step_stride, std::vector<hipEvent_t>* evs = nullptr);
int build_graph(rdx_ctx* c, void* scores, bool fixed = false);
```

### radialog_amd/csrc/rdx_kernels.h

```cpp
#pragma once
#include <hip/hip_runtime.h>
#include <stdint.h>

namespace rdx {

enum Epilogue {
    EPI_NONE = 0,
    EPI_RELU = 1,
    EPI_GELU = 2,
    EPI_RESID = 3,
    EPI_SILU_MUL = 4,
    EPI_LOGITS = 5,
    EPI_RESID_RELU = 6,
};

enum ActLayout : int {
    ACT_ROWS = 0,
    ACT_BLK32 = 1,
    ACT_BLK64 = 2,
    ACT_TILES32 = 3,
    ACT_BLK64_E4M3 = 4,
    ACT_ROWS_E4M3 = 5,
};

struct GemmArgs {
    const void* X; int ldx;
    const void* W;
    const float* bias;
    const void* resid; int ldr;
    void* out; int ldo;
    int M, N, K;
    const void* norm_w; float eps;
    float* part_val; int* part_idx;
    int n_valid;
    const int* out_step; long out_step_stride;
    const void* W8; const float* wscale;
    ActLayout out_packed;
    ActLayout xpacked;
    int mtiles;
    int xdup_off;
    const float* xscale; int xgroups;
    long long* trace;
};

struct ConvGeom {
    int mode;
    int Hin, Win, Cin, Hout, Wout, KH, KW, stride, pad;
};

struct PConvArgs {
    const void* X; const void* W; const float* bias; const void* resid; void* out;
    const void* zero16;
    int Hin, Win, Cin, Hout, Wout, N;
    int M;
    int mt_in, mt_out;
    int ldo;
    int clog;
    int no_ksplit;
    int tile_m, tile_n, tile_k;
};

struct AttnArgs {
    const void* Q; const void* K; const void* V; void* O;
    long q_bs, q_ts, q_hs;
    long k_bs, k_ts, k_hs;
    long v_bs, v_ts, v_hs;
    long o_bs, o_ts, o_hs;
    int B, H, Tq, Tk;
    int causal;
    int k_perm;
    const uint8_t* key_mask; long km_bs;
    int flash_min;
    int o_packed_mt;
};


// ... 55 lines not shown
                      int packed_mt, hipStream_t s);

void launch_l2_bench(int mode, const void* buf, size_t bytes_per_wg, int shared, int reps, int wgs, unsigned* sink, hipStream_t s);

void launch_attention(int dtype, int head_dim, const AttnArgs& a, hipStream_t s);
bool flash_prefill_supported(int head_dim, const AttnArgs& a);
void launch_flash_prefill(int dtype, const AttnArgs& a, hipStream_t s);
void launch_rope_kv_prefill(int dtype, const LlamaDims& d, const void* qkv, const void* lora_bq, const void* lora_bv,
                            const void* cos_t, const void* sin_t, const int* pos_ids, void* qout, void* kcache,
                            void* vcache, int B, int T, int slot0, hipStream_t s);
void launch_k_unperm(const void* kc, void* out, size_t slabs, int max_len, int perm, hipStream_t s);
struct DecAttnArgs {
    LlamaDims d;
    const void *qkv, *lbq, *lbv, *cos_t, *sin_t;
    const void* cur_rope = nullptr;
    const int *pos, *slot_b;
    const uint8_t* key_mask;
    void *kcache, *vcache, *out;
    long long* trace = nullptr;
    ActLayout out_packed = ACT_ROWS;
    int out_mt = 2;
    const int* epoch = nullptr;
    int layers = 0, layer = 0;
};
void launch_decode_attention(int dtype, const DecAttnArgs& a, int B, hipStream_t s);
struct ChainArgs {
    const void *wdown, *wqkv;
    const void *wdown8, *wqkv8;
    const float *sdown, *sqkv;
    const void* attn_norm;
    int layer;
    int hidden, inter, qkv_n, qkv_ld, B;
    int w8;
    float eps;
    void *dx, *dqkv, *dgu;
    int* ctr;
    int* err;
    int naps;
    long long* trace;
};
bool chain_supported(const LlamaDims& d, int inter, int B);
size_t chain_ctr_ints(int layers);
void launch_decode_chain(int dtype, ChainArgs ca, bool with_next_qkv, hipStream_t s);
constexpr int HO_HINT_INTS = 128;
bool attn_oproj16_supported(const LlamaDims& d, int N, int K, int B);
void launch_attn_oproj16(int dtype, const DecAttnArgs& a, const GemmArgs& g, int B, int* hint, int* err, hipStream_t s);

struct NormArgs {
    void* x; const void* w;
    void* out; float* xscale;
    int rows, H; float eps;
    ActLayout layout; int mtiles;
    const float* slab; int groups;
};
bool rmsnorm_supported(const NormArgs& n);
bool launch_rmsnorm(int dtype, const NormArgs& n, hipStream_t s);
void launch_quant_rows(int dtype, const void* x, long ldx, void* out8, float* xscale, int rows, int K, int groups, hipStream_t s);
bool gemm8_supported(const GemmArgs& a, int epi);
void launch_gemm8(int dtype, const GemmArgs& a, int epi, hipStream_t s);
void launch_layernorm(int dtype, const void* x, const float* gamma, const float* beta, void* out, float* out_f32,
                      int rows, int H, float eps, hipStream_t s);
void launch_layernorm_ex(int dtype, const void* x, long ldx, const float* gamma, const float* beta, const void* emb, int emb_rows,
                         void* out, long ldo, int rows, int H, float eps, hipStream_t s);
void launch_pool_gather(int dtype, const void* src, void* dst, int B, int L, int C, hipStream_t s);
void launch_pool_concat(int dtype, const void* patch, const void* tokens, void* dst, int B, int L, int C, hipStream_t s);
void launch_scramble_layernorm(int dtype, const void* pp_nhwc, const float* gamma, const float* beta, void* out,
// ... 54 lines not shown
```

### radialog_amd/csrc/skinny_body.h

```cpp
#pragma once
#include "rdx_common.h"
#include "rdx_kernels.h"
#include "handoff.h"

namespace rdx {

template <typename T> __device__ __forceinline__ float swiglu(float gate_acc, float up_acc) {
    const float gt = rnd<T>(gate_acc), up = rnd<T>(up_acc);
    const float s = rnd<T>(silu(gt));
    return s * up;
}


template <typename T, int MT, int EPI, bool NORM, int WAVES, bool XLDS, typename WaitFn, bool COHX = false, bool W8 = false, typename Late>
__device__ __forceinline__ void skinny_tile(const void* Wb, const int K, const int tile, const int ntiles, unsigned char* dyn_smem,
                                            WaitFn wait_inputs, Late late) {
    typedef typename Vec8<T>::type V8;
    static_assert(!W8 || (XLDS && MT == 1), "fp8 weights: LDS-staged activations, one M tile");
    constexpr int U = (XLDS && WAVES >= 8) ? 8 : 4;
    constexpr int NTHR = WAVES * 64;
    __shared__ __attribute__((aligned(16))) float red[WAVES][MT][256];
    __shared__ float ssq[WAVES][16];
    __shared__ float rstd_s[16];
    T* xs = reinterpret_cast<T*>(dyn_smem);

    const int lane = threadIdx.x & 63, w = __builtin_amdgcn_readfirstlane(threadIdx.x >> 6);
    const int r = lane & 15, g = lane >> 4;
    const int KC = W8 ? (K >> 6) : (K >> 5);
    const int c0 = (KC * w) / WAVES, c1 = (KC * (w + 1)) / WAVES;
    const u4* wbase = reinterpret_cast<const u4*>(Wb) + (size_t)tile * KC * 64 + lane;
    const int clast = min(max(c1 - 1, c0), KC - 1);

    const long long t_entry = (long long)__builtin_amdgcn_s_memrealtime();
    u4 ring[2 * U];
#pragma unroll
    for (int u = 0; u < 2 * U; ++u) ring[u] = ldg16_nt(wbase + (size_t)min(c0 + u, clast) * 64);
    u4* const wv = ring;
    u4* const wn = ring + U;
    __builtin_amdgcn_sched_barrier(0);
    const GemmArgs a = late();
    const T* X = reinterpret_cast<const T*>(a.X);

    long long* trc = (a.trace && threadIdx.x == 0) ? a.trace + (size_t)tile * 8 : nullptr;
#define SK_T(i) do { if (trc) trc[i] = (long long)__builtin_amdgcn_s_memrealtime(); } while (0)
    if (trc) {
        trc[0] = t_entry;
        trc[6] = (long long)__builtin_amdgcn_s_getreg((4 << 0) | (0 << 6) | (31 << 11));
        trc[7] = (long long)__builtin_amdgcn_s_getreg((20 << 0) | (0 << 6) | (31 << 11));
    }

    SK_T(1);
    wait_inputs();

    auto ldxa = [&](const T* p) -> u4 {
        if (!COHX) return ldg16(p);
        const unsigned long long lo = ld8_agent(p), hi = ld8_agent(p + 4);
        return (u4){(unsigned)lo, (unsigned)(lo >> 32), (unsigned)hi, (unsigned)(hi >> 32)};
    };
    if (XLDS) {
        const int K8 = K >> 3;
        if (NORM) {
            for (int m = 0; m < a.M; ++m) {
                float ss = 0.f;
                for (int k8 = threadIdx.x; k8 < K8; k8 += NTHR) {
                    V8 xv = as_vec8<T>(ldxa(X + (size_t)m * a.ldx + (size_t)k8 * 8));
#pragma unroll
                    for (int j = 0; j < 8; ++j) { const float f = tof<T>(xv[j]); ss += f * f; }
                }
                ss = wave_sum(ss);
                if (lane == 0) ssq[w][m] = ss;
            }
            __syncthreads();
            if (threadIdx.x < a.M) {
                float t = 0.f;
#pragma unroll
                for (int i = 0; i < WAVES; ++i) t += ssq[i][threadIdx.x];
                rstd_s[threadIdx.x] = rsqrtf(t / (float)K + a.eps);
            }
            __syncthreads();
        }
        const T* NW = reinterpret_cast<const T*>(a.norm_w);
        const int total8 = a.M * K8;
        for (int i = threadIdx.x; i < total8; i += NTHR) {
            const int m = i / K8, k8 = i - m * K8;
            V8 xv = as_vec8<T>(ldxa(X + (size_t)m * a.ldx + (size_t)k8 * 8));
            if (NORM) {
                const float rs = rstd_s[m];
                V8 nw = as_vec8<T>(ldg16(NW + (size_t)k8 * 8));
#pragma unroll
                for (int j = 0; j < 8; ++j) {
                    const float h = rnd<T>(tof<T>(xv[j]) * rs);
                    xv[j] = fromf<T>(tof<T>(nw[j]) * h);
                }
            }
            *reinterpret_cast<u4*>(xs + (size_t)m * K + (size_t)k8 * 8) = as_u4<T>(xv);
        }
        __syncthreads();
    }

    SK_T(2);
    const T* xrow[MT];
    bool xok[MT];
#pragma unroll
    for (int mt = 0; mt < MT; ++mt) {
        const int m = mt * 16 + r;
        xok[mt] = m < a.M;
        xrow[mt] = XLDS ? (xs + (size_t)(xok[mt] ? m : 0) * K + g * (W8 ? 16 : 8)) : (X + (size_t)(xok[mt] ? m : 0) * a.ldx + g * 8);
    }

    v4f acc[MT];
#pragma unroll
    for (int mt = 0; mt < MT; ++mt) acc[mt] = (v4f){0.f, 0.f, 0.f, 0.f};

    u4 xr[U][MT], xn[U][MT];
    auto load_x = [&](u4 (&dst)[U][MT], int cb) {
#pragma unroll
        for (int u = 0; u < U; ++u) {
            const int c = min(cb + u, clast);
#pragma unroll
            for (int mt = 0; mt < MT; ++mt)
                dst[u][mt] = xok[mt] ? ldxa(xrow[mt] + (size_t)c * 32) : (u4){0u, 0u, 0u, 0u};
        }
    };
    if (!XLDS) load_x(xr, c0);

    if (XLDS) {
        auto consume1 = [&](const u4& wreg, int c) {
            if (W8) {
#pragma unroll
                for (int h = 0; h < 2; ++h) {
                    const u4 wd = dequant8<T>(h ? wreg.z : wreg.x, h ? wreg.w : wreg.y);
                    const u4 xv = *reinterpret_cast<const u4*>(xrow[0] + (size_t)c * 64 + h * 8);
                    acc[0] = mfma16(as_vec8<T>(wd), as_vec8<T>(xv), acc[0]);
                }
            } else {
#pragma unroll
                for (int mt = 0; mt < MT; ++mt) {
                    const u4 xv = *reinterpret_cast<const u4*>(xrow[mt] + (size_t)c * 32);
                    acc[mt] = mfma16(as_vec8<T>(wreg), as_vec8<T>(xv), acc[mt]);
                }
            }
        };
        int cb = c0;
        for (; cb + 2 * U < c1; cb += 2 * U) {
#pragma unroll
            for (int u = 0; u < 2 * U; ++u) {
                consume1(ring[u], cb + u);
                ring[u] = ldg16_nt(wbase + (size_t)min(cb + 2 * U + u, clast) * 64);
                __builtin_amdgcn_sched_barrier(0);
            }
        }
#pragma unroll
        for (int u = 0; u < 2 * U; ++u)
            if (cb + u < c1) consume1(ring[u], cb + u);
    } else
    for (int cb = c0; cb < c1; cb += U) {
        if (!XLDS && cb + U < c1) load_x(xn, cb + U);
#pragma unroll
        for (int u = 0; u < U; ++u) {
            if (W8) {
                if (cb + u < c1) {
#pragma unroll
                    for (int h = 0; h < 2; ++h) {
                        const u4 wd = dequant8<T>(h ? wv[u].z : wv[u].x, h ? wv[u].w : wv[u].y);
                        const u4 xv = xok[0] ? *reinterpret_cast<const u4*>(xrow[0] + (size_t)(cb + u) * 64 + h * 8) : (u4){0u, 0u, 0u, 0u};
                        acc[0] = mfma16(as_vec8<T>(wd), as_vec8<T>(xv), acc[0]);
                    }
                }
            } else if (cb + u < c1) {
#pragma unroll
                for (int mt = 0; mt < MT; ++mt) {
                    u4 xv;
                    if (XLDS) xv = xok[mt] ? *reinterpret_cast<const u4*>(xrow[mt] + (size_t)(cb + u) * 32) : (u4){0u, 0u, 0u, 0u};
                    else xv = xr[u][mt];
                    acc[mt] = mfma16(as_vec8<T>(wv[u]), as_vec8<T>(xv), acc[mt]);
                }
            }
        }
#pragma unroll
        for (int u = 0; u < U; ++u) wv[u] = wn[u];
        if (!XLDS && cb + U < c1) {
#pragma unroll
            for (int u = 0; u < U; ++u)
#pragma unroll
                for (int mt = 0; mt < MT; ++mt) xr[u][mt] = xn[u][mt];
        }
        if (cb + 2 * U < c1) {
// ... 67 lines not shown
```

### radialog_amd/engine.py

```python
from __future__ import annotations

import ctypes as C
import math
import numbers
from dataclasses import dataclass
from typing import Callable, Dict, Optional

import torch

from . import _lib
from ._lib import RdxConfig, check
from .config import RaDialogCfg
from . import weights as W

_TORCH_DT = {"f16": torch.float16, "bf16": torch.bfloat16}
_RDX_DT = {"f16": _lib.RDX_DTYPE_F16, "bf16": _lib.RDX_DTYPE_BF16}


def _ptr(t: Optional[torch.Tensor]):
    return None if t is None else C.c_void_p(t.data_ptr())


@dataclass(frozen=True)
class LogitsRules:
# ... 440 lines not shown

    def logits_test(self, x, w, n_valid=None, fp8=False):
        import ctypes
        M, K = x.shape
        N = w.shape[0]
        x = x.to(self.device, self.tdtype).contiguous()
        w = w.to(self.device, torch.float32).contiguous()
        out = torch.zeros(M, N, dtype=self.tdtype, device=self.device)
        am = (ctypes.c_int32 * M)()
        torch.cuda.synchronize(self.device)
        check(self.ctx, self.lib.rdx_logits_test(self.ctx, _ptr(x), _ptr(w), M, N, N if n_valid is None else n_valid, K, _ptr(out),
                                                 ctypes.cast(am, ctypes.c_void_p), int(fp8)), "rdx_logits_test")
        return out, torch.tensor(list(am), dtype=torch.int32)

    def _dev(self, t, dtype=None):
        return None if t is None else t.to(self.device, dtype or self.tdtype).contiguous()

    def _nan(self, *shape, dtype=None):
        return torch.full(shape, float("nan"), dtype=dtype or self.tdtype, device=self.device)

    def xstat16_test(self, x, norm_w, w, epi=0, eps=1e-6, n_valid=None, ldo=None, out_packed=0):
        import ctypes
        M, N = x.shape[0], w.shape[0]
        x, nw, w = self._dev(x), self._dev(norm_w), self._dev(w, torch.float32)
        cols = N // 2 if epi == 4 else N
        ldo = ldo or cols
        out = self._nan(N // 64, 2, 64, 8) if out_packed else self._nan(M + 2, ldo)
        am = (ctypes.c_int32 * M)()
        torch.cuda.synchronize(self.device)
        check(self.ctx, self.lib.rdx_xstat16_test(self.ctx, _ptr(x), _ptr(nw), eps, _ptr(w), M, N, epi, N if n_valid is None else n_valid, _ptr(out),
                                                  ldo, out_packed, ctypes.cast(am, ctypes.c_void_p)), "rdx_xstat16_test")
        return (out, torch.tensor(list(am), dtype=torch.int32)) if epi == 5 else out

    def xrow16_test(self, x, w, resid, M=None, ldo=None):
        packed = x.dim() == 4
        M = M if packed else x.shape[0]
        N, K = w.shape
        x, w, r = self._dev(x), self._dev(w, torch.float32), self._dev(resid)
        ldo = ldo or N
        out = self._nan(M + 2, ldo)
        torch.cuda.synchronize(self.device)
        check(self.ctx, self.lib.rdx_xrow16_test(self.ctx, _ptr(x), int(packed), _ptr(w), _ptr(r), M, N, K, _ptr(out), ldo), "rdx_xrow16_test")
        return out

    def xstat_blk_test(self, x, norm_w, w, epi=0, resid=None, eps=1e-6, n_valid=None, ldo=None, out_packed=0, want_xp=False):
        import ctypes
        M, N = x.shape[0], w.shape[0]
        mtl = (M + 15) // 16
        x, nw, w, r = self._dev(x), self._dev(norm_w), self._dev(w, torch.float32), self._dev(resid)
        ldo = ldo or (N // 2 if epi == 4 else N)
        out = self._nan(N // 64, mtl, 64, 8) if out_packed else self._nan(M + 2, ldo)
        xp = self._nan(128, mtl, 64, 8) if want_xp else None
        am = (ctypes.c_int32 * M)()
        torch.cuda.synchronize(self.device)
        check(self.ctx, self.lib.rdx_xstat_blk_test(self.ctx, _ptr(x), _ptr(nw), eps, _ptr(w), _ptr(r), M, N, epi, N if n_valid is None else n_valid,
                                                    _ptr(out), ldo, out_packed, _ptr(xp), ctypes.cast(am, ctypes.c_void_p)), "rdx_xstat_blk_test")
        return out, xp, (torch.tensor(list(am), dtype=torch.int32) if epi == 5 else None)

    def xsplit_blk_test(self, x, w, resid=None, norm_w=None, eps=1e-6):
        M, N = x.shape[0], w.shape[0]
        mtl = (M + 15) // 16
        x, w, nw = self._dev(x), self._dev(w, torch.float32), self._dev(norm_w)
        slab = self._nan(4, 16 * mtl, N, dtype=torch.float32)
        r = None if resid is None else self._dev(resid).clone()
        xn = None if resid is None else self._nan(128, mtl, 64, 8)
        torch.cuda.synchronize(self.device)
# ... 164 lines not shown
```

Measured before the change: 1.569 reports/s.

## Add lossless 13-bit coded bf16 weight format for decode GEMV and chain kernels

At context creation, lm_head, gate/up, down and qkv weights are re-encoded into a compact form. Each tile stores the low 8 bits per element, a 4-bit exponent index relative to a per-tile base exponent, and a sign plane. The decode skinny GEMV and the fused decode chain read these 52-byte-per-lane chunks and rebuild exact bf16 fragments before the MFMA. The goal is to cut HBM weight traffic in the memory-bound batch-1 decode. Tiles whose exponents do not fit the 15-step window fall back to the raw weights, which costs extra decode ALU work, an extra device copy of the weights and more code paths.

Result: faster. 1.664 reports/s (median of 6 runs) (+6.1%).

```diff
diff --git a/include/rdx_dec_hooks.h b/include/rdx_dec_hooks.h
--- a/include/rdx_dec_hooks.h
+++ b/include/rdx_dec_hooks.h
@@ -40,6 +40,9 @@
                     const rdx_logits_rules* rules, int eos_id, const rdx_sampling* sampling, int32_t* tokens_out);
 int rdx_sample_u24_host(uint64_t seed, uint32_t row, uint32_t draw, uint32_t* out);
 
+int rdx_wcode_test(rdx_ctx* ctx, const float* W, int N, int K, void* packed_out, void* planes_out, uint32_t* hdr_out);
+int rdx_wcode_stats(rdx_ctx* ctx, long long* out);
+
 #ifdef __cplusplus
 }
 #endif
diff --git a/radialog_amd/_lib.py b/radialog_amd/_lib.py
--- a/radialog_amd/_lib.py
+++ b/radialog_amd/_lib.py
@@ -122,6 +122,8 @@
     "rdx_decode_attn_test": (C.c_int, [_P, C.c_int, C.c_int, C.c_int, C.c_int, C.c_int, _F, _P, _P, _P, _P, _P, _P, C.c_int, _P, _P, _P, _P, _P, _P, C.c_longlong,
                                        C.c_int, C.c_int]),
     "rdx_rope_kv_test": (C.c_int, [_P, C.c_int, C.c_int, C.c_int, C.c_int, C.c_int, C.c_int, _F, _P, _P, _P, _P, _P, C.c_int, _P, C.c_int, _P, _P, _P]),
+    "rdx_wcode_test": (C.c_int, [_P, _P, C.c_int, C.c_int, _P, _P, _P]),
+    "rdx_wcode_stats": (C.c_int, [_P, C.POINTER(C.c_longlong)]),
 }
 ALL_HOOK_SYMBOLS = {**HOOK_SYMBOLS, **ENC_HOOK_SYMBOLS, **DEC_HOOK_SYMBOLS}
 
diff --git a/radialog_amd/csrc/api.hip b/radialog_amd/csrc/api.hip
--- a/radialog_amd/csrc/api.hip
+++ b/radialog_amd/csrc/api.hip
@@ -225,6 +225,24 @@
             }
         }
         if (R.rc) return R.rc;
+        const bool fp8_mode = fp8_weights(c->ll[0].wqkv) || fp8_weights(c->ll[0].wgu) || fp8_weights(c->lm_head);
+        LlamaDims probe = {}; probe.hidden = H; probe.heads = f.heads; probe.head_dim = 128;
+        if (f.dtype == DT_BF16 && !fp8_mode && H % WC_CHUNK_K == 0 && I % WC_CHUNK_K == 0 && chain_supported(probe, I, 1)) {
+            auto encode = [&](GemmW& W) -> int {
+                if (!W.w || W.wc) return 0;
+                ALLOC(c, W.wc, wc_bytes(W.Npad, W.K));
+                ALLOC(c, W.wch, (size_t)(W.Npad / 16) * sizeof(unsigned));
+                launch_encode_wc(W.w, W.wc, W.wch, W.Npad, W.K, c->stream);
+                return 0;
+            };
+            if (int erc = encode(c->lm_head)) return erc;
+            for (int l = 0; l < f.layers; ++l) {
+                if (l > 0) if (int erc = encode(c->ll[l].wqkv)) return erc;
+                if (int erc = encode(c->ll[l].wgu)) return erc;
+                if (int erc = encode(c->ll[l].wdown)) return erc;
+            }
+            HIPCHK(c, hipStreamSynchronize(c->stream));
+        }
         c->ld.hidden = H; c->ld.heads = f.heads; c->ld.head_dim = 128; c->ld.qkv_ld = c->ll[0].wqkv.Npad;
         c->ld.lora_r = f.lora_r; c->ld.lora_scale = f.lora_scale; c->ld.max_len = f.max_len; c->ld.max_pos = f.max_pos;
         c->ld.k_perm = (getenv("RDX_KPERM") ? atoi(getenv("RDX_KPERM")) : (f.max_batch * f.heads <= 256)) ? 1 : 0;
@@ -351,5 +369,10 @@
         if (c->graph) { hipGraphExecDestroy(c->graph); c->graph = nullptr; c->gkey = GraphKey(); }
         return 0;
     }
+    if (!strcmp(name, "wcode")) {
+        c->wcode = value != 0;
+        if (c->graph) { hipGraphExecDestroy(c->graph); c->graph = nullptr; c->gkey = GraphKey(); }
+        return 0;
+    }
     return fail(c, -1, "rdx_set_option: unknown option '%s'", name);
 }
diff --git a/radialog_amd/csrc/api_debug.hip b/radialog_amd/csrc/api_debug.hip
--- a/radialog_amd/csrc/api_debug.hip
+++ b/radialog_amd/csrc/api_debug.hip
@@ -71,6 +71,7 @@
     if (what != 1 && what != 2) { a.out = c->dqkv; a.resid = nullptr; a.ldr = 0; }
     if ((a.N + 15) / 16 > max_tiles) { hipFree(dtr); return fail(c, -1, "rdx_gemv_trace: need room for %d tiles", (a.N + 15) / 16); }
     a.trace = dtr;
+    if (what == 1) a = coded_unit(c, a, L.wgu, B);
     skinny(c, a, what == 1 ? EPI_SILU_MUL : EPI_NONE);
     hipError_t e = hipStreamSynchronize(c->stream);
     if (e == hipSuccess) e = hipMemcpy(host, dtr, bytes, hipMemcpyDeviceToHost);
@@ -229,13 +230,28 @@
 extern "C" int rdx_gemm_test(rdx_ctx* c, const void* X, const float* W, const float* bias, const void* resid, void* out,
                              int M, int N, int K, int epi, const void* norm_w, float eps, int force) {
     if (!c || !X || !W || !out) return fail(c, -1, "rdx_gemm_test: null argument");
-    if (K % 32 || N % 16) return fail(c, -1, "rdx_gemm_test: need K %% 32 == 0 and N %% 16 == 0");
+    const bool gemv = force == 1 || force == 12;
+    if (K % 32 || (N % 16 && !gemv) || N <= 0) return fail(c, -1, "rdx_gemm_test: need K %% 32 == 0 and N %% 16 == 0");
     HIPCHK(c, hipSetDevice(c->device));
     GemmW w;
-    w.N = N; w.K = K; w.Npad = N;
+    w.N = N; w.K = K; w.Npad = (N + 15) / 16 * 16;
     void* wp = nullptr;
-    HIPCHK(c, hipMalloc(&wp, (size_t)N * K * 2 + ((force == 4 || (force >= 9 && force <= 11)) ? (size_t)N * K + (size_t)N * 4 : 0)));
+    HIPCHK(c, hipMalloc(&wp, (size_t)w.Npad * K * 2 + ((force == 4 || (force >= 9 && force <= 11)) ? (size_t)N * K + (size_t)N * 4 : 0)));
     w.w = wp;
+    struct Coded {
+        void* planes = nullptr; unsigned* hdr = nullptr;
+        ~Coded() { if (planes) hipFree(planes); if (hdr) hipFree(hdr); }
+    } coded;
+    if (force == 12) {
+        if (c->cfg.dtype != DT_BF16 || K % WC_CHUNK_K || M >= xs_min_rows() || !skinny_fits_lds(M, K)) {
+            hipFree(wp);
+            return fail(c, -1, "rdx_gemm_test: force 12 (coded bf16 weights) needs a bf16 context, K %% 128 == 0 and M <= 2 rows that fit the GEMV's LDS stage");
+        }
+        if (hipMalloc(&coded.planes, wc_bytes(w.Npad, K)) != hipSuccess || hipMalloc((void**)&coded.hdr, (size_t)(w.Npad / 16) * sizeof(unsigned)) != hipSuccess) {
+            hipFree(wp);
+            return fail(c, -2, "rdx_gemm_test: out of device memory");
+        }
+    }
     if (force >= 9 && force <= 11) {
         const int G = force == 9 ? 1 : (force == 10 ? 2 : 4);
         if (K % 64 || (norm_w && G != 1)) { hipFree(wp); return fail(c, -1, "rdx_gemm_test: gemm8 needs K %% 64 == 0 (and one K group behind an RMSNorm)"); }
@@ -267,10 +283,16 @@
         launch_pack_weight_fp8(c->cfg.dtype, W, w.w8, w.scale, nullptr, N, K, N, c->stream);
         force = 1;
     } else
-    launch_pack_weight(c->cfg.dtype, W, wp, N, K, N, nullptr, c->stream);
+    launch_pack_weight(c->cfg.dtype, W, wp, N, K, w.Npad, nullptr, c->stream);
     GemmArgs a = gargs(X, K, w, bias, out, epi == EPI_SILU_MUL ? N / 2 : N, M);
     a.resid = resid; a.ldr = N;
     a.norm_w = norm_w; a.eps = eps;
+    if (force == 12) {
+        launch_encode_wc(wp, coded.planes, coded.hdr, w.Npad, K, c->stream);
+        a.WC = coded.planes; a.wchdr = coded.hdr;
+        if (epi == EPI_LOGITS || !skinny_wc_supported(c->cfg.dtype, a, epi)) { hipFree(wp); return fail(c, -1, "rdx_gemm_test: force 12: no coded GEMV for epilogue %d", epi); }
+        force = 1;
+    }
     void* xn = nullptr;
     bool split8 = false;
     if (force == 6) {
@@ -366,13 +388,18 @@
 extern "C" int rdx_logits_test(rdx_ctx* c, const void* X, const float* W, int M, int N, int n_valid, int K, void* out_logits,
                                int32_t* argmax_host, int fp8) {
     if (!c || !X || !W || !out_logits || !argmax_host) return fail(c, -1, "rdx_logits_test: null argument");
+    const bool coded = fp8 == 2;
+    if (coded) fp8 = 0;
     if (K % 32 || N % 16 || M > 32 || n_valid > N || (fp8 && K % 64)) return fail(c, -1, "rdx_logits_test: bad shape");
+    if (coded && (c->cfg.dtype != DT_BF16 || K % WC_CHUNK_K || M >= xs_min_rows() || !skinny_fits_lds(M, K)))
+        return fail(c, -1, "rdx_logits_test: coded bf16 weights need a bf16 context, K %% 128 == 0 and M <= 2 rows that fit the GEMV's LDS stage");
     HIPCHK(c, hipSetDevice(c->device));
     GemmW w;
     w.N = N; w.K = K; w.Npad = N;
     const int nt = N / 16;
     char* wp = nullptr;
-    const size_t wb = (size_t)N * K * 2, qb = fp8 ? (size_t)N * K + (size_t)N * 4 : 0, pb = (size_t)M * nt * 4;
+    const size_t cpb = coded ? wc_bytes(N, K) : 0;
+    const size_t wb = (size_t)N * K * 2, qb = fp8 ? (size_t)N * K + (size_t)N * 4 : cpb + (coded ? (size_t)nt * 4 : 0), pb = (size_t)M * nt * 4;
     HIPCHK(c, hipMalloc((void**)&wp, wb + qb + 2 * pb + (size_t)M * K * 2));
     w.w = wp;
     if (fp8) {
@@ -384,6 +411,10 @@
     GemmArgs a = gargs(X, K, w, nullptr, out_logits, N, M);
     a.n_valid = n_valid;
     a.part_val = (float*)(wp + wb + qb); a.part_idx = (int*)(wp + wb + qb + pb);
+    if (coded) {
+        launch_encode_wc(wp, wp + wb, (unsigned*)(wp + wb + cpb), N, K, c->stream);
+        a.WC = wp + wb; a.wchdr = (const unsigned*)(wp + wb + cpb);
+    }
     char* blk = nullptr;
     int brc = fp8_block_for_test(c, a, EPI_LOGITS, &blk);
     if (brc) { hipFree(wp); return brc; }
diff --git a/radialog_amd/csrc/api_dec_hooks.hip b/radialog_amd/csrc/api_dec_hooks.hip
--- a/radialog_amd/csrc/api_dec_hooks.hip
+++ b/radialog_amd/csrc/api_dec_hooks.hip
@@ -342,3 +342,36 @@
     *out = sample_u24(seed, row, draw);
     return 0;
 }
+
+extern "C" int rdx_wcode_test(rdx_ctx* c, const float* W, int N, int K, void* packed_out, void* planes_out, uint32_t* hdr_out) {
+    if (!c || !W || !packed_out || !planes_out || !hdr_out || N <= 0 || K <= 0) return fail(c, -1, "rdx_wcode_test: bad arguments");
+    if (c->cfg.dtype != DT_BF16 || K % WC_CHUNK_K) return fail(c, -1, "rdx_wcode_test: coded weights need a bf16 context and K %% 128 == 0");
+    HIPCHK(c, hipSetDevice(c->device));
+    const int npad = (N + 15) / 16 * 16;
+    launch_pack_weight(c->cfg.dtype, W, packed_out, N, K, npad, nullptr, c->stream);
+    launch_encode_wc(packed_out, planes_out, hdr_out, npad, K, c->stream);
+    return finish(c);
+}
+
+extern "C" int rdx_wcode_stats(rdx_ctx* c, long long* out) {
+    if (!c || !out || !c->finalized) return fail(c, -1, "rdx_wcode_stats: a finalized context and an output are needed");
+    HIPCHK(c, hipSetDevice(c->device));
+    HIPCHK(c, hipStreamSynchronize(c->stream));
+    out[0] = out[1] = out[2] = 0;
+    out[3] = c->n_wc_gemv; out[4] = c->n_wc_chain;
+    std::vector<const GemmW*> ws;
+    if (c->cfg.enable_llama) {
+        ws.push_back(&c->lm_head);
+        for (const LlamaLayer& L : c->ll) { ws.push_back(&L.wqkv); ws.push_back(&L.wo); ws.push_back(&L.wgu); ws.push_back(&L.wdown); }
+    }
+    for (const GemmW* W : ws) {
+        if (!W->wc || !W->wch) continue;
+        const int nt = W->Npad / 16;
+        std::vector<unsigned> h(nt);
+        HIPCHK(c, hipMemcpy(h.data(), W->wch, (size_t)nt * sizeof(unsigned), hipMemcpyDeviceToHost));
+        out[0] += nt;
+        for (unsigned v : h) out[1] += (v >> 8) & 1u;
+        out[2] += (long long)wc_bytes(W->Npad, W->K) + (long long)nt * 4;
+    }
+    return 0;
+}
diff --git a/radialog_amd/csrc/api_dispatch.hip b/radialog_amd/csrc/api_dispatch.hip
--- a/radialog_amd/csrc/api_dispatch.hip
+++ b/radialog_amd/csrc/api_dispatch.hip
@@ -49,6 +49,11 @@
     return a;
 }
 
+GemmArgs coded_unit(rdx_ctx* c, GemmArgs a, const GemmW& W, int B) {
+    if (c->wcode && W.wc && W.wch && decode_family(c, B) == DEC_CHAINED) { a.WC = W.wc; a.wchdr = W.wch; }
+    return a;
+}
+
 GemmArgs xs16_unit(rdx_ctx* c, const LlamaLayer* L, DecUnit u, int B) {
     GemmArgs a = unit_args(c, L, u, B);
     if (u == UNIT_GATE_UP) a.out_packed = ACT_BLK32;
@@ -125,6 +130,7 @@
             return;
         }
     }
+    if (skinny_wc_supported(c->cfg.dtype, a, epi) && !xstat32_supported(a, epi)) ++c->n_wc_gemv;
     launch_skinny_gemm(c->cfg.dtype, a, epi, c->stream);
 }
 
diff --git a/radialog_amd/csrc/api_inspect.hip b/radialog_amd/csrc/api_inspect.hip
--- a/radialog_amd/csrc/api_inspect.hip
+++ b/radialog_amd/csrc/api_inspect.hip
@@ -97,6 +97,7 @@
                     else skinny(c, a, EPI_NONE);
                 } else {
                     GemmArgs a = unit_args(c, L, u, B);
+                    if (u != UNIT_QKV) a = coded_unit(c, a, u == UNIT_GATE_UP ? L->wgu : c->lm_head, B);
                     if (hoisted) { a = prenormed(c, a); a.xpacked = pn.xpacked; a.xscale = pn.xscale; a.xgroups = pn.xgroups; }
                     launch_skinny_gemm(dt, a, epi, c->stream);
                 }
diff --git a/radialog_amd/csrc/api_llama.hip b/radialog_amd/csrc/api_llama.hip
--- a/radialog_amd/csrc/api_llama.hip
+++ b/radialog_amd/csrc/api_llama.hip
@@ -35,7 +35,11 @@
     case DEC_XS16:
         if (x == c->dx) { launch_xstat16(f.dtype, lm(xs16_unit(c, nullptr, UNIT_LM_HEAD, B)), EPI_LOGITS, c->stream); break; }
         [[fallthrough]];
-    default: skinny(c, lm(unit_args(c, nullptr, UNIT_LM_HEAD, B)), EPI_LOGITS);
+    default: {
+        GemmArgs a = lm(unit_args(c, nullptr, UNIT_LM_HEAD, B));
+        if (advance) a = coded_unit(c, a, c->lm_head, B);
+        skinny(c, a, EPI_LOGITS);
+    }
     }
     StepTail t = {};
     t.eos_id = c->cur_eos; t.pad_id = c->cur_pad; t.max_new = c->cur_max_new; t.out_tokens = c->cur_tokens; t.unfinished = c->d_unf;
@@ -337,7 +341,7 @@
     skinny(c, unit_args(c, &L0, UNIT_QKV, B), EPI_NONE);
     for (int l = 0; l < f.layers; ++l) {
         attn_oproj(c, l, B);
-        skinny(c, unit_args(c, &c->ll[l], UNIT_GATE_UP, B), EPI_SILU_MUL);
+        skinny(c, coded_unit(c, unit_args(c, &c->ll[l], UNIT_GATE_UP, B), c->ll[l].wgu, B), EPI_SILU_MUL);
         mark();
         ca.layer = l;
         {
@@ -346,6 +350,10 @@
             ca.wdown = L.wdown.w; ca.wdown8 = L.wdown.w8; ca.sdown = L.wdown.scale;
             ca.wqkv = Ln ? Ln->wqkv.w : nullptr; ca.wqkv8 = Ln ? Ln->wqkv.w8 : nullptr; ca.sqkv = Ln ? Ln->wqkv.scale : nullptr;
             ca.attn_norm = Ln ? Ln->attn_norm : nullptr;
+            ca.wc = (c->wcode && !ca.w8 && L.wdown.wc && L.wdown.wch && (!Ln || (Ln->wqkv.wc && Ln->wqkv.wch))) ? 1 : 0;
+            ca.cdown = L.wdown.wc; ca.hdown = L.wdown.wch;
+            ca.cqkv = Ln ? Ln->wqkv.wc : nullptr; ca.hqkv = Ln ? Ln->wqkv.wch : nullptr;
+            if (ca.wc && f.dtype == DT_BF16) ++c->n_wc_chain;
         }
         ca.trace = l == c->chain_trace_layer ? c->chain_trace : nullptr;
         launch_decode_chain(f.dtype, ca, l + 1 < f.layers, s);
diff --git a/radialog_amd/csrc/chain.hip b/radialog_amd/csrc/chain.hip
--- a/radialog_amd/csrc/chain.hip
+++ b/radialog_amd/csrc/chain.hip
@@ -19,9 +19,9 @@
     const float* wscale;
 };
 
-template <typename WaitFn> struct ChainLate { ChainGemm a; WaitFn wait; long long* trace; };
-
-template <typename T, int EPI, bool NORM, int SUB, int XL, typename WaitFn, int U = 4, bool RESID_EARLY = false, bool W8 = false, typename Late>
+template <typename WaitFn> struct ChainLate { ChainGemm a; WaitFn wait; long long* trace; const void* wraw = nullptr; const unsigned* wchdr = nullptr; };
+
+template <typename T, int EPI, bool NORM, int SUB, int XL, typename WaitFn, int U = 4, bool RESID_EARLY = false, bool W8 = false, bool WC = false, typename Late>
 __device__ __forceinline__ ChainLate<WaitFn> chain_tile(const void* Wb, const int K, const int wg, const int ntiles, unsigned char* smem, Late late) {
     typedef typename Vec8<T>::type V8;
     constexpr int WPS = CH_WAVES / SUB;
@@ -39,24 +39,37 @@
     const int c0 = (KC * w) / WPS, c1 = (KC * (w + 1)) / WPS;
     const u4* wbase = reinterpret_cast<const u4*>(Wb) + (size_t)tile_c * KC * 64 + lane;
     const int clast = min(max(c1 - 1, c0), KC - 1);
+    static_assert(!WC || (!W8 && U % 2 == 0), "coded weights: model dtype");
+    constexpr int RC = U / 2;
+    const int KQ = K >> 7, q0 = c0 >> 2, q1 = c1 > c0 ? (c1 + 3) >> 2 : q0, qlast = min(max(q1 - 1, q0), KQ - 1);
+    const unsigned char* cb16 = reinterpret_cast<const unsigned char*>(Wb) + (size_t)tile_c * KQ * WC_CHUNK_BYTES + lane * 16;
+    const unsigned char* cb4 = reinterpret_cast<const unsigned char*>(Wb) + (size_t)tile_c * KQ * WC_CHUNK_BYTES + 3072 + lane * 4;
     const long long t_entry = (long long)__builtin_amdgcn_s_memrealtime();
 
     u4 wa_[U], wb_[U];
-#pragma unroll
-    for (int u = 0; u < U; ++u) wa_[u] = ldg16_nt(wbase + (size_t)min(c0 + u, clast) * 64);
-#pragma unroll
-    for (int u = 0; u < U; ++u) wb_[u] = ldg16_nt(wbase + (size_t)min(c0 + U + u, clast) * 64);
+    WcChunk cring[RC];
+    if constexpr (WC) {
+#pragma unroll
+        for (int u = 0; u < RC; ++u) { const size_t o = (size_t)min(q0 + u, qlast) * WC_CHUNK_BYTES; cring[u] = wc_load(cb16 + o, cb4 + o); }
+    } else {
+#pragma unroll
+        for (int u = 0; u < U; ++u) wa_[u] = ldg16_nt(wbase + (size_t)min(c0 + u, clast) * 64);
+#pragma unroll
+        for (int u = 0; u < U; ++u) wb_[u] = ldg16_nt(wbase + (size_t)min(c0 + U + u, clast) * 64);
+    }
     __builtin_amdgcn_sched_barrier(0);
     const ChainLate<WaitFn> lt = late();
     const ChainGemm& a = lt.a;
     const WaitFn& wait_inputs = lt.wait;
     long long* const trace = lt.trace;
+    unsigned wc_hdr = 0;
+    if constexpr (WC) wc_hdr = *(reinterpret_cast<const __attribute__((address_space(4))) unsigned*>((uintptr_t)lt.wchdr) + tile_c);
     const T* X = reinterpret_cast<const T*>(a.X);
     long long* trc = (trace && threadIdx.x == 0) ? trace : nullptr;
 #define CH_T(i) do { if (trc) trc[i] = (long long)__builtin_amdgcn_s_memrealtime(); } while (0)
     if (trc) trc[0] = t_entry;
     if (trace) {
-        if (threadIdx.x < 64) asm volatile("s_waitcnt vmcnt(%0)" :: "n"(2 * U - 1) : "memory");
+        if (threadIdx.x < 64) asm volatile("s_waitcnt vmcnt(%0)" :: "n"(WC ? 4 * RC - 1 : 2 * U - 1) : "memory");
         CH_T(5);
     }
 
@@ -136,6 +149,7 @@
                 *reinterpret_cast<unsigned long long*>(xs + (size_t)m * K + (size_t)k4 * 4) = v;
             }
         }
+        if (WC && threadIdx.x == 0) *reinterpret_cast<u4*>(xs + (size_t)a.M * K) = (u4){0u, 0u, 0u, 0u};
         __syncthreads();
     }
 
@@ -173,18 +187,66 @@
             acc = mfma16(as_vec8<T>(wv), as_vec8<T>(xv), acc);
         }
     };
-    int cb = c0;
-    for (; cb + 2 * U < c1; cb += 2 * U) {
-#pragma unroll
-        for (int u = 0; u < 2 * U; ++u) {
-            u4& wr = u < U ? wa_[u] : wb_[u - U];
-            consume1(wr, cb + u);
-            wr = ldg16_nt(wbase + (size_t)min(cb + 2 * U + u, clast) * 64);
-            __builtin_amdgcn_sched_barrier(0);
-        }
-    }
-    consume(wa_, cb, true);
-    consume(wb_, cb + U, true);
+    if constexpr (WC) {
+        if (wc_hdr & 0x100u) {
+            const u4* wraw = reinterpret_cast<const u4*>(lt.wraw) + (size_t)tile_c * KC * 64 + lane;
+            auto slot = [&](int u) -> u4& { return u == 0 ? cring[0].lo0 : u == 1 ? cring[0].lo1 : u == 2 ? cring[0].ix : cring[1].lo0; };
+#pragma unroll
+            for (int u = 0; u < 4; ++u) slot(u) = ldg16_nt(wraw + (size_t)min(c0 + u, clast) * 64);
+            int cb = c0;
+            for (; cb + 4 < c1; cb += 4) {
+#pragma unroll
+                for (int u = 0; u < 4; ++u) {
+                    consume1(slot(u), cb + u);
+                    slot(u) = ldg16_nt(wraw + (size_t)min(cb + 4 + u, clast) * 64);
+                    __builtin_amdgcn_sched_barrier(0);
+                }
+            }
+#pragma unroll
+            for (int u = 0; u < 4; ++u)
+                if (cb + u < c1) consume1(slot(u), cb + u);
+        } else {
+            const unsigned base4 = (wc_hdr & 0xffu) * 0x01010101u;
+            const T* zptr = xs + (size_t)a.M * K;
+            auto consumeC = [&](const WcChunk& ch, int q, bool guard) {
+                auto one = [&](const u4 wd, int c) {
+                    const T* xp = (!guard || (c >= c0 && c < c1)) ? xrow + (size_t)c * 32 : zptr;
+                    acc = mfma16(as_vec8<T>(wd), as_vec8<T>(*reinterpret_cast<const u4*>(xp)), acc);
+                    __builtin_amdgcn_sched_barrier(0);
+                };
+                one(wc_frag<0>(ch, base4), 4 * q); one(wc_frag<1>(ch, base4), 4 * q + 1);
+                one(wc_frag<2>(ch, base4), 4 * q + 2); one(wc_frag<3>(ch, base4), 4 * q + 3);
+            };
+            auto trip = [&](int q, bool guard) {
+#pragma unroll
+                for (int u = 0; u < RC; ++u) {
+                    consumeC(cring[u], q + u, guard);
+                    const size_t o = (size_t)min(q + RC + u, qlast) * WC_CHUNK_BYTES;
+                    cring[u] = wc_load(cb16 + o, cb4 + o);
+                    __builtin_amdgcn_sched_barrier(0);
+                }
+            };
+            int q = q0;
+            if (q + RC < q1) { trip(q, true); q += RC; }
+            for (; q + RC < q1; q += RC) trip(q, false);
+#pragma unroll
+            for (int u = 0; u < RC; ++u)
+                if (q + u < q1) consumeC(cring[u], q + u, true);
+        }
+    } else {
+        int cb = c0;
+        for (; cb + 2 * U < c1; cb += 2 * U) {
+    #pragma unroll
+            for (int u = 0; u < 2 * U; ++u) {
+                u4& wr = u < U ? wa_[u] : wb_[u - U];
+                consume1(wr, cb + u);
+                wr = ldg16_nt(wbase + (size_t)min(cb + 2 * U + u, clast) * 64);
+                __builtin_amdgcn_sched_barrier(0);
+            }
+        }
+        consume(wa_, cb, true);
+        consume(wb_, cb + U, true);
+    }
     CH_T(1);
     *reinterpret_cast<float4*>(&red[wa * 256 + r * 16 + g * 4]) = make_float4(acc[0], acc[1], acc[2], acc[3]);
     __syncthreads();
@@ -259,6 +321,30 @@
         int* ctr = ca.ctr + (size_t)ca.layer * HO_CTR_INTS;
         return ChainLate<WaitSharded>{ChainGemm{ca.dx, H, nullptr, 0, ca.dqkv, ca.qkv_ld, ca.B, qkv_n, ca.attn_norm, ca.eps, ca.sqkv},
                                       WaitSharded{ctr, nwg_down, ca.err, ca.naps, nullptr}, ca.trace ? ca.trace + (size_t)blockIdx.x * 8 : nullptr};
+    });
+}
+
+__global__ __launch_bounds__(CH_THREADS, 4) void decode_chain_wc_k(const void* cdown, const void* cqkv, int hidden, int inter, int qkv_n, int nwg_down, ChainArgs) {
+    extern __shared__ __attribute__((aligned(16))) unsigned char msm[];
+    typedef bf16 T;
+    const int H = hidden;
+    auto args = [] { return late_kernarg<ChainArgs>(kernarg_offset<6>(decltype(&decode_chain_wc_k){})); };
+    if ((int)blockIdx.x < nwg_down) {
+        const ChainLate<WaitSharded> lt = chain_tile<T, EPI_RESID, false, 1, 6, WaitSharded, 4, false, false, true>(cdown, inter, blockIdx.x, nwg_down, msm, [&] {
+            const ChainArgs ca = args();
+            int* ctr = ca.ctr + (size_t)ca.layer * HO_CTR_INTS;
+            return ChainLate<WaitSharded>{ChainGemm{ca.dgu, inter, ca.dx, H, ca.dx, H, ca.B, H, nullptr, 0.f, nullptr},
+                                          WaitSharded{ctr, 0, ca.err, ca.naps, nullptr}, ca.trace ? ca.trace + (size_t)blockIdx.x * 8 : nullptr, ca.wdown, ca.hdown};
+        });
+        publish_sc1(lt.wait.ctr, blockIdx.x);
+        if (lt.trace && threadIdx.x == 0) lt.trace[2] = (long long)__builtin_amdgcn_s_memrealtime();
+        return;
+    }
+    chain_tile<T, EPI_NONE, true, 4, 2, WaitSharded, 8, false, false, true>(cqkv, H, blockIdx.x - nwg_down, (qkv_n + 15) / 16, msm, [&] {
+        const ChainArgs ca = args();
+        int* ctr = ca.ctr + (size_t)ca.layer * HO_CTR_INTS;
+        return ChainLate<WaitSharded>{ChainGemm{ca.dx, H, nullptr, 0, ca.dqkv, ca.qkv_ld, ca.B, qkv_n, ca.attn_norm, ca.eps, nullptr},
+                                      WaitSharded{ctr, nwg_down, ca.err, ca.naps, nullptr}, ca.trace ? ca.trace + (size_t)blockIdx.x * 8 : nullptr, ca.wqkv, ca.hqkv};
     });
 }
 
@@ -328,7 +414,7 @@
     const int nwg_down = ca.hidden / 16;
     const int nwg_qkv = with_next_qkv ? ((ca.qkv_n + 15) / 16 + 3) / 4 : 0;
     const int kmax = ca.inter > ca.hidden ? ca.inter : ca.hidden;
-    const size_t sm_gemm = (size_t)(CH_WAVES * 256 + CH_WAVES * CH_MAXM + 16) * 4 + (size_t)ca.B * kmax * 2;
+    const size_t sm_gemm = (size_t)(CH_WAVES * 256 + CH_WAVES * CH_MAXM + 16) * 4 + (size_t)ca.B * kmax * 2 + 16;
     const size_t smem = sm_gemm > (size_t)84 * 1024 ? sm_gemm : (size_t)84 * 1024;
     dim3 grid(nwg_down + nwg_qkv), block(CH_THREADS);
     RDX_DISPATCH_T(dtype, T, {
@@ -337,7 +423,11 @@
             hipFuncSetAttribute((const void*)decode_chain_k<T, false>, hipFuncAttributeMaxDynamicSharedMemorySize, 100 * 1024);
             hipFuncSetAttribute((const void*)decode_chain_k<T, true>, hipFuncAttributeMaxDynamicSharedMemorySize, 100 * 1024);
         }
-        if (ca.w8) hipLaunchKernelGGL((decode_chain_k<T, true>), grid, block, smem, s, ca.wdown8, ca.wqkv8, ca.hidden, ca.inter, ca.qkv_n, nwg_down, ca);
+        if (ca.wc && dtype == DT_BF16 && !ca.w8) {
+            static DevOnce wc_attr_set;
+            if (wc_attr_set.first()) hipFuncSetAttribute((const void*)decode_chain_wc_k, hipFuncAttributeMaxDynamicSharedMemorySize, 100 * 1024);
+            hipLaunchKernelGGL(decode_chain_wc_k, grid, block, smem, s, ca.cdown, with_next_qkv ? ca.cqkv : ca.cdown, ca.hidden, ca.inter, ca.qkv_n, nwg_down, ca);
+        } else if (ca.w8) hipLaunchKernelGGL((decode_chain_k<T, true>), grid, block, smem, s, ca.wdown8, ca.wqkv8, ca.hidden, ca.inter, ca.qkv_n, nwg_down, ca);
         else hipLaunchKernelGGL((decode_chain_k<T, false>), grid, block, smem, s, ca.wdown, ca.wqkv, ca.hidden, ca.inter, ca.qkv_n, nwg_down, ca);
     });
 }
diff --git a/radialog_amd/csrc/gemm.hip b/radialog_amd/csrc/gemm.hip
--- a/radialog_amd/csrc/gemm.hip
+++ b/radialog_amd/csrc/gemm.hip
@@ -85,6 +85,60 @@
                                                 scale, (T*)dst, N, K, Npad));
 }
 
+__global__ __launch_bounds__(256) void encode_wc_k(const u4* __restrict__ packed, unsigned char* __restrict__ planes, unsigned* __restrict__ hdr, int K) {
+    __shared__ int s_top, s_raw;
+    const int tile = blockIdx.x, KC = K >> 5, KQ = K >> 7, lane = threadIdx.x & 63, wv = threadIdx.x >> 6;
+    if (threadIdx.x == 0) { s_top = 0; s_raw = 0; }
+    __syncthreads();
+    const u4* src = packed + (size_t)tile * KC * 64;
+    int top = 0, bad = 0;
+    for (int i = threadIdx.x; i < KC * 64; i += 256) {
+        const u4 v = src[i];
+#pragma unroll
+        for (int d = 0; d < 4; ++d)
+#pragma unroll
+            for (int hlf = 0; hlf < 2; ++hlf) {
+                const int h = (int)((v[d] >> (16 * hlf + 8)) & 0x7fu);
+                if (h == 127) bad = 1; else top = max(top, h);
+            }
+    }
+    atomicMax(&s_top, top);
+    if (bad) atomicOr(&s_raw, 1);
+    __syncthreads();
+    const int base = max(s_top - 15, 0);
+    for (int q = wv; q < KQ; q += 4) {
+        unsigned lo[8], ix[4], sg = 0;
+#pragma unroll
+        for (int j = 0; j < 4; ++j) {
+            const u4 v = src[(size_t)(4 * q + j) * 64 + lane];
+            unsigned l0 = 0, l1 = 0, n = 0;
+#pragma unroll
+            for (int e = 0; e < 8; ++e) {
+                const unsigned wbits = (v[e >> 1] >> (16 * (e & 1))) & 0xffffu;
+                const int h = (int)((wbits >> 8) & 0x7fu);
+                int idx = h ? h - base : 0;
+                if (h && (idx < 1 || idx > 15)) { bad = 1; idx = 0; }
+                if (e < 4) l0 |= (wbits & 0xffu) << (8 * e); else l1 |= (wbits & 0xffu) << (8 * (e - 4));
+                n |= (unsigned)idx << (4 * (e < 4 ? 2 * e : 2 * (e - 4) + 1));
+                sg |= (wbits >> 15) << ((2 * j + (e >> 2)) + 8 * (e & 3));
+            }
+            lo[2 * j] = l0; lo[2 * j + 1] = l1; ix[j] = n;
+        }
+        unsigned char* p = planes + ((size_t)tile * KQ + q) * WC_CHUNK_BYTES;
+        reinterpret_cast<u4*>(p)[lane] = (u4){lo[0], lo[1], lo[2], lo[3]};
+        reinterpret_cast<u4*>(p + 1024)[lane] = (u4){lo[4], lo[5], lo[6], lo[7]};
+        reinterpret_cast<u4*>(p + 2048)[lane] = (u4){ix[0], ix[1], ix[2], ix[3]};
+        reinterpret_cast<unsigned*>(p + 3072)[lane] = sg;
+    }
+    if (bad) atomicOr(&s_raw, 1);
+    __syncthreads();
+    if (threadIdx.x == 0) hdr[tile] = (unsigned)base | (s_raw ? 0x100u : 0u);
+}
+
+void launch_encode_wc(const void* packed, void* planes, unsigned* hdr, int npad, int K, hipStream_t s) {
+    hipLaunchKernelGGL(encode_wc_k, dim3(npad / 16), dim3(256), 0, s, (const u4*)packed, (unsigned char*)planes, hdr, K);
+}
+
 template <typename T, int MT, int EPI, bool NORM, int WAVES, bool XLDS, bool W8 = false>
 __global__ __launch_bounds__(WAVES * 64, WAVES == 4 ? 8 : 1) void skinny_gemm_k(const void* Wb, const void* X, int K, int N, GemmArgs) {
     extern __shared__ __attribute__((aligned(16))) unsigned char dyn_smem[];
@@ -94,6 +148,37 @@
         a.X = X; a.K = K; a.N = N;
         return a;
     });
+}
+
+template <int EPI, bool NORM, int WAVES>
+__global__ __launch_bounds__(WAVES * 64, WAVES == 4 ? 8 : 1) void skinny_gemm_wc_k(const void* Wc, const void* X, int K, int N, const unsigned* hdr, GemmArgs) {
+    extern __shared__ __attribute__((aligned(16))) unsigned char dyn_smem[];
+    skinny_tile<bf16, 1, EPI, NORM, WAVES, true, NoWait, false, false, true>(Wc, K, blockIdx.x, (N + 15) / 16, dyn_smem, NoWait(), [&] {
+        constexpr unsigned off = kernarg_offset<5>(decltype(&skinny_gemm_wc_k<EPI, NORM, WAVES>){});
+        GemmArgs a = late_kernarg<GemmArgs>(off);
+        a.X = X; a.K = K; a.N = N;
+        return a;
+    }, hdr);
+}
+
+template <bool NORM, int WAVES>
+static void launch_skinny_wc(const GemmArgs& a, int epi, hipStream_t s) {
+    dim3 grid((a.N + 15) / 16), block(WAVES * 64);
+    const size_t dyn = (size_t)a.M * a.K * 2 + 16;
+#define RDX_SKC(E) hipLaunchKernelGGL((skinny_gemm_wc_k<E, NORM, WAVES>), grid, block, dyn, s, a.WC, a.X, a.K, a.N, a.wchdr, a)
+    switch (epi) {
+        case EPI_NONE: RDX_SKC(EPI_NONE); break;
+        case EPI_RESID: RDX_SKC(EPI_RESID); break;
+        case EPI_SILU_MUL: RDX_SKC(EPI_SILU_MUL); break;
+        case EPI_LOGITS: RDX_SKC(EPI_LOGITS); break;
+        default: break;
+    }
+#undef RDX_SKC
+}
+
+bool skinny_wc_supported(int dtype, const GemmArgs& a, int epi) {
+    return dtype == DT_BF16 && a.WC && a.wchdr && a.W && skinny_fits_lds(a.M, a.K) && a.K % WC_CHUNK_K == 0 && a.M < xs_min_rows() &&
+           (epi == EPI_NONE || epi == EPI_RESID || epi == EPI_SILU_MUL || epi == EPI_LOGITS);
 }
 
 template <typename T, int MT, bool NORM, int WAVES, bool XLDS, bool W8 = false>
@@ -116,19 +201,27 @@
 
 bool skinny_fits_lds(int M, int K) { return M <= 16 && (size_t)M * K * 2 <= 32 * 1024; }
 
+static int skinny_lds_waves(const GemmArgs& a) {
+    const int nt = (a.N + 15) / 16;
+    if (nt <= 256 && a.K >= 4096) return 16;
+    if (nt > 512 && (size_t)a.M * a.K * 2 <= 16 * 1024) return 4;
+    return 8;
+}
+
 template <typename T>
 static void launch_skinny_T(const GemmArgs& a, int epi, hipStream_t s) {
     const bool norm = a.norm_w != nullptr;
     constexpr int WV = 8;
     constexpr bool wide = true;
     const bool w8 = a.W8 && a.wscale && skinny_fits_lds(a.M, a.K) && a.K % 64 == 0;
-    if (wide && skinny_fits_lds(a.M, a.K) && (a.N + 15) / 16 <= 256 && a.K >= 4096) {
+    const int lds_waves = skinny_fits_lds(a.M, a.K) ? skinny_lds_waves(a) : 0;
+    if (wide && lds_waves == 16) {
         if (w8) { if (norm) launch_skinny_epi<T, 1, true, 16, true, true>(a, epi, s); else launch_skinny_epi<T, 1, false, 16, true, true>(a, epi, s); return; }
         if (norm) launch_skinny_epi<T, 1, true, 16, true>(a, epi, s); else launch_skinny_epi<T, 1, false, 16, true>(a, epi, s);
         return;
     }
     constexpr bool smallwg = true;
-    if (smallwg && skinny_fits_lds(a.M, a.K) && (a.N + 15) / 16 > 512 && (size_t)a.M * a.K * 2 <= 16 * 1024) {
+    if (smallwg && lds_waves == 4) {
         if (w8) { if (norm) launch_skinny_epi<T, 1, true, 4, true, true>(a, epi, s); else launch_skinny_epi<T, 1, false, 4, true, true>(a, epi, s); return; }
         if (norm) launch_skinny_epi<T, 1, true, 4, true>(a, epi, s); else launch_skinny_epi<T, 1, false, 4, true>(a, epi, s);
         return;
@@ -145,6 +238,14 @@
 
 void launch_skinny_gemm(int dtype, const GemmArgs& a, int epi, hipStream_t s) {
     if (xstat32_supported(a, epi) && (!(a.W8 && a.wscale) || (a.xpacked == ACT_BLK64_E4M3 && a.xscale))) { launch_xstat32(dtype, a, epi, s); return; }
+    if (skinny_wc_supported(dtype, a, epi)) {
+        const bool norm = a.norm_w != nullptr;
+        const int waves = skinny_lds_waves(a);
+        if (waves == 16) { if (norm) launch_skinny_wc<true, 16>(a, epi, s); else launch_skinny_wc<false, 16>(a, epi, s); }
+        else if (waves == 4) { if (norm) launch_skinny_wc<true, 4>(a, epi, s); else launch_skinny_wc<false, 4>(a, epi, s); }
+        else { if (norm) launch_skinny_wc<true, 8>(a, epi, s); else launch_skinny_wc<false, 8>(a, epi, s); }
+        return;
+    }
     RDX_DISPATCH_T(dtype, T, launch_skinny_T<T>(a, epi, s));
 }
 
diff --git a/radialog_amd/csrc/rdx_common.h b/radialog_amd/csrc/rdx_common.h
--- a/radialog_amd/csrc/rdx_common.h
+++ b/radialog_amd/csrc/rdx_common.h
@@ -73,6 +73,27 @@
                 __builtin_bit_cast(unsigned, __builtin_amdgcn_cvt_pkrtz(c[0], c[1])), __builtin_bit_cast(unsigned, __builtin_amdgcn_cvt_pkrtz(d[0], d[1]))};
 }
 
+struct WcChunk { u4 lo0, lo1, ix; unsigned sg; };
+__device__ __forceinline__ unsigned ldg4_nt(const void* p) { return __builtin_nontemporal_load((const __attribute__((address_space(1))) unsigned*)p); }
+__device__ __forceinline__ WcChunk wc_load(const unsigned char* p16, const unsigned char* p4) {
+    WcChunk c;
+    c.lo0 = ldg16_nt(p16); c.lo1 = ldg16_nt(p16 + 1024); c.ix = ldg16_nt(p16 + 2048); c.sg = ldg4_nt(p4);
+    return c;
+}
+template <int GI> __device__ __forceinline__ unsigned wc_hi4(unsigned x, unsigned base4, unsigned sg) {
+    const unsigned m = (x + 0x7f7f7f7fu) & 0x80808080u;
+    const unsigned keep = m - (m >> 7);
+    return ((x + base4) & keep) | ((sg << (7 - GI)) & 0x80808080u);
+}
+template <int J> __device__ __forceinline__ u4 wc_frag(const WcChunk& c, unsigned base4) {
+    const unsigned n = c.ix[J];
+    const u4& lo = J < 2 ? c.lo0 : c.lo1;
+    const unsigned l0 = lo[2 * (J & 1)], l1 = lo[2 * (J & 1) + 1];
+    const unsigned h0 = wc_hi4<2 * J>(n & 0x0f0f0f0fu, base4, c.sg), h1 = wc_hi4<2 * J + 1>((n >> 4) & 0x0f0f0f0fu, base4, c.sg);
+    return (u4){__builtin_amdgcn_perm(h0, l0, 0x05010400u), __builtin_amdgcn_perm(h0, l0, 0x07030602u),
+                __builtin_amdgcn_perm(h1, l1, 0x05010400u), __builtin_amdgcn_perm(h1, l1, 0x07030602u)};
+}
+
 __device__ __forceinline__ void fp8_scale(float amax, float& sc, float& inv) {
     sc = amax > 0.f ? amax / 448.0f : 1.0f;
     inv = amax > 0.f ? 448.0f / amax : 1.0f;
diff --git a/radialog_amd/csrc/rdx_ctx.h b/radialog_amd/csrc/rdx_ctx.h
--- a/radialog_amd/csrc/rdx_ctx.h
+++ b/radialog_amd/csrc/rdx_ctx.h
@@ -18,7 +18,10 @@
 
 constexpr int RDX_MAX_ROWS = 128;
 
-struct GemmW { void* w = nullptr; int N = 0, K = 0, Npad = 0; void* w8 = nullptr; float* scale = nullptr; };
+struct GemmW {
+    void* w = nullptr; int N = 0, K = 0, Npad = 0; void* w8 = nullptr; float* scale = nullptr;
+    void* wc = nullptr; unsigned* wch = nullptr;
+};
 struct RawW { void* p = nullptr; int64_t rows = 0, cols = 0; };
 
 struct LlamaLayer {
@@ -96,6 +99,8 @@
     bool xs16 = true;
     bool prompt_blk = true;
     bool blk_down = true;
+    bool wcode = true;
+    long long n_wc_gemv = 0, n_wc_chain = 0;
     int chain_naps = 1;
     long long* chain_trace = nullptr; int chain_trace_layer = -1;
     long long* ao_trace = nullptr; int ao_trace_layer = -1;
@@ -177,6 +182,7 @@
 DecAttnArgs dec_attn_args(rdx_ctx* c, int layer);
 AttnArgs prefill_attn_args(rdx_ctx* c, int B, int T, int keep, int layer);
 GemmArgs unit_args(rdx_ctx* c, const LlamaLayer* L, DecUnit u, int B);
+GemmArgs coded_unit(rdx_ctx* c, GemmArgs a, const GemmW& W, int B);
 GemmArgs xs16_unit(rdx_ctx* c, const LlamaLayer* L, DecUnit u, int B);
 GemmArgs blk_unit(rdx_ctx* c, const LlamaLayer* L, DecUnit u, int B);
 GemmArgs blk8_unit(rdx_ctx* c, const LlamaLayer* L, DecUnit u, int B);
diff --git a/radialog_amd/csrc/rdx_kernels.h b/radialog_amd/csrc/rdx_kernels.h
--- a/radialog_amd/csrc/rdx_kernels.h
+++ b/radialog_amd/csrc/rdx_kernels.h
@@ -41,7 +41,13 @@
     int xdup_off;
     const float* xscale; int xgroups;
     long long* trace;
-};
+    const void* WC; const unsigned* wchdr;
+};
+
+constexpr int WC_CHUNK_K = 128, WC_CHUNK_BYTES = 64 * 52;
+inline size_t wc_bytes(int npad, int k) { return (size_t)(npad / 16) * (size_t)(k / WC_CHUNK_K) * WC_CHUNK_BYTES; }
+void launch_encode_wc(const void* packed, void* planes, unsigned* hdr, int npad, int K, hipStream_t s);
+bool skinny_wc_supported(int dtype, const GemmArgs& a, int epi);
 
 struct ConvGeom {
     int mode;
@@ -163,6 +169,7 @@
     int layer;
     int hidden, inter, qkv_n, qkv_ld, B;
     int w8;
+    const void *cdown, *cqkv; const unsigned *hdown, *hqkv; int wc;
     float eps;
     void *dx, *dqkv, *dgu;
     int* ctr;
diff --git a/radialog_amd/csrc/skinny_body.h b/radialog_amd/csrc/skinny_body.h
--- a/radialog_amd/csrc/skinny_body.h
+++ b/radialog_amd/csrc/skinny_body.h
@@ -2,6 +2,7 @@
 #include "rdx_common.h"
 #include "rdx_kernels.h"
 #include "handoff.h"
+#include <type_traits>
 
 namespace rdx {
 
@@ -12,11 +13,13 @@
 }
 
 
-template <typename T, int MT, int EPI, bool NORM, int WAVES, bool XLDS, typename WaitFn, bool COHX = false, bool W8 = false, typename Late>
+template <typename T, int MT, int EPI, bool NORM, int WAVES, bool XLDS, typename WaitFn, bool COHX = false, bool W8 = false, bool WC = false, typename Late>
 __device__ __forceinline__ void skinny_tile(const void* Wb, const int K, const int tile, const int ntiles, unsigned char* dyn_smem,
-                                            WaitFn wait_inputs, Late late) {
+                                            WaitFn wait_inputs, Late late, const unsigned* wchdr = nullptr) {
     typedef typename Vec8<T>::type V8;
     static_assert(!W8 || (XLDS && MT == 1), "fp8 weights: LDS-staged activations, one M tile");
+    static_assert(!WC || (XLDS && MT == 1 && !W8), "coded weights: LDS-staged activations, one M tile, model dtype");
+    constexpr int R = 2;
     constexpr int U = (XLDS && WAVES >= 8) ? 8 : 4;
     constexpr int NTHR = WAVES * 64;
     __shared__ __attribute__((aligned(16))) float red[WAVES][MT][256];
@@ -30,16 +33,27 @@
     const int c0 = (KC * w) / WAVES, c1 = (KC * (w + 1)) / WAVES;
     const u4* wbase = reinterpret_cast<const u4*>(Wb) + (size_t)tile * KC * 64 + lane;
     const int clast = min(max(c1 - 1, c0), KC - 1);
+    const int KQ = K >> 7, q0 = c0 >> 2, q1 = c1 > c0 ? (c1 + 3) >> 2 : q0, qlast = min(max(q1 - 1, q0), KQ - 1);
+    const unsigned char* cb16 = reinterpret_cast<const unsigned char*>(Wb) + (size_t)tile * KQ * WC_CHUNK_BYTES + lane * 16;
+    const unsigned char* cb4 = reinterpret_cast<const unsigned char*>(Wb) + (size_t)tile * KQ * WC_CHUNK_BYTES + 3072 + lane * 4;
 
     const long long t_entry = (long long)__builtin_amdgcn_s_memrealtime();
     u4 ring[2 * U];
-#pragma unroll
-    for (int u = 0; u < 2 * U; ++u) ring[u] = ldg16_nt(wbase + (size_t)min(c0 + u, clast) * 64);
+    WcChunk cring[R];
+    if constexpr (WC) {
+#pragma unroll
+        for (int u = 0; u < R; ++u) { const size_t o = (size_t)min(q0 + u, qlast) * WC_CHUNK_BYTES; cring[u] = wc_load(cb16 + o, cb4 + o); }
+    } else {
+#pragma unroll
+        for (int u = 0; u < 2 * U; ++u) ring[u] = ldg16_nt(wbase + (size_t)min(c0 + u, clast) * 64);
+    }
     u4* const wv = ring;
     u4* const wn = ring + U;
     __builtin_amdgcn_sched_barrier(0);
     const GemmArgs a = late();
     const T* X = reinterpret_cast<const T*>(a.X);
+    unsigned wc_hdr = 0;
+    if constexpr (WC) wc_hdr = *(reinterpret_cast<const __attribute__((address_space(4))) unsigned*>((uintptr_t)wchdr) + tile);
 
     long long* trc = (a.trace && threadIdx.x == 0) ? a.trace + (size_t)tile * 8 : nullptr;
 #define SK_T(i) do { if (trc) trc[i] = (long long)__builtin_amdgcn_s_memrealtime(); } while (0)
@@ -95,6 +109,7 @@
             }
             *reinterpret_cast<u4*>(xs + (size_t)m * K + (size_t)k8 * 8) = as_u4<T>(xv);
         }
+        if (WC && threadIdx.x == 0) *reinterpret_cast<u4*>(xs + (size_t)a.M * K) = (u4){0u, 0u, 0u, 0u};
         __syncthreads();
     }
 
@@ -141,18 +156,59 @@
                 }
             }
         };
-        int cb = c0;
-        for (; cb + 2 * U < c1; cb += 2 * U) {
-#pragma unroll
-            for (int u = 0; u < 2 * U; ++u) {
-                consume1(ring[u], cb + u);
-                ring[u] = ldg16_nt(wbase + (size_t)min(cb + 2 * U + u, clast) * 64);
-                __builtin_amdgcn_sched_barrier(0);
-            }
-        }
-#pragma unroll
-        for (int u = 0; u < 2 * U; ++u)
-            if (cb + u < c1) consume1(ring[u], cb + u);
+        auto raw_loop = [&](const u4* wb, auto slot, auto nr) {
+            constexpr int NR = decltype(nr)::value;
+            int cb = c0;
+            for (; cb + NR < c1; cb += NR) {
+#pragma unroll
+                for (int u = 0; u < NR; ++u) {
+                    consume1(slot(u), cb + u);
+                    slot(u) = ldg16_nt(wb + (size_t)min(cb + NR + u, clast) * 64);
+                    __builtin_amdgcn_sched_barrier(0);
+                }
+            }
+#pragma unroll
+            for (int u = 0; u < NR; ++u)
+                if (cb + u < c1) consume1(slot(u), cb + u);
+        };
+        if constexpr (WC) {
+            if (wc_hdr & 0x100u) {
+                const u4* wraw = reinterpret_cast<const u4*>(a.W) + (size_t)tile * KC * 64 + lane;
+                auto slot = [&](int u) -> u4& { return u == 0 ? cring[0].lo0 : u == 1 ? cring[0].lo1 : u == 2 ? cring[0].ix : cring[1].lo0; };
+#pragma unroll
+                for (int u = 0; u < 4; ++u) slot(u) = ldg16_nt(wraw + (size_t)min(c0 + u, clast) * 64);
+                raw_loop(wraw, slot, std::integral_constant<int, 4>());
+            } else {
+                const unsigned base4 = (wc_hdr & 0xffu) * 0x01010101u;
+                const T* zptr = xs + (size_t)a.M * K;
+                auto consumeC = [&](const WcChunk& ch, int q, bool guard) {
+                    auto one = [&](const u4 wd, int c) {
+                        const T* xp = (!guard || (c >= c0 && c < c1)) ? xrow[0] + (size_t)c * 32 : zptr;
+                        acc[0] = mfma16(as_vec8<T>(wd), as_vec8<T>(*reinterpret_cast<const u4*>(xp)), acc[0]);
+                        __builtin_amdgcn_sched_barrier(0);
+                    };
+                    one(wc_frag<0>(ch, base4), 4 * q); one(wc_frag<1>(ch, base4), 4 * q + 1);
+                    one(wc_frag<2>(ch, base4), 4 * q + 2); one(wc_frag<3>(ch, base4), 4 * q + 3);
+                };
+                auto trip = [&](int q, bool guard) {
+#pragma unroll
+                    for (int u = 0; u < R; ++u) {
+                        consumeC(cring[u], q + u, guard);
+                        const size_t o = (size_t)min(q + R + u, qlast) * WC_CHUNK_BYTES;
+                        cring[u] = wc_load(cb16 + o, cb4 + o);
+                        __builtin_amdgcn_sched_barrier(0);
+                    }
+                };
+                int q = q0;
+                if (q + R < q1) { trip(q, true); q += R; }
+                for (; q + R < q1; q += R) trip(q, false);
+#pragma unroll
+                for (int u = 0; u < R; ++u)
+                    if (q + u < q1) consumeC(cring[u], q + u, true);
+            }
+        } else {
+            raw_loop(wbase, [&](int u) -> u4& { return ring[u]; }, std::integral_constant<int, 2 * U>());
+        }
     } else
     for (int cb = c0; cb < c1; cb += U) {
         if (!XLDS && cb + U < c1) load_x(xn, cb + U);
diff --git a/radialog_amd/engine.py b/radialog_amd/engine.py
--- a/radialog_amd/engine.py
+++ b/radialog_amd/engine.py
@@ -496,6 +496,23 @@
                                                   ldo, out_packed, ctypes.cast(am, ctypes.c_void_p)), "rdx_xstat16_test")
         return (out, torch.tensor(list(am), dtype=torch.int32)) if epi == 5 else out
 
+    def wcode_test(self, w):
+        from . import wcode
+        N, K = w.shape
+        nt = (N + 15) // 16
+        w = self._dev(w, torch.float32)
+        packed = torch.zeros(nt, K // 32, 64, 8, dtype=torch.int16, device=self.device)
+        planes = torch.zeros(nt, K // wcode.CHUNK_K, wcode.CHUNK_BYTES, dtype=torch.uint8, device=self.device)
+        hdr = torch.zeros(nt, dtype=torch.int32, device=self.device)
+        torch.cuda.synchronize(self.device)
+        check(self.ctx, self.lib.rdx_wcode_test(self.ctx, _ptr(w), N, K, _ptr(packed), _ptr(planes), _ptr(hdr)), "rdx_wcode_test")
+        return packed.cpu().numpy().view("uint16"), planes.cpu().numpy(), hdr.cpu().numpy().view("uint32")
+
+    def wcode_stats(self):
+        out = (C.c_longlong * 5)()
+        check(self.ctx, self.lib.rdx_wcode_stats(self.ctx, out), "rdx_wcode_stats")
+        return tuple(int(v) for v in out)
+
     def xrow16_test(self, x, w, resid, M=None, ldo=None):
         packed = x.dim() == 4
         M = M if packed else x.shape[0]
diff --git a/radialog_amd/wcode.py b/radialog_amd/wcode.py
--- /dev/null
+++ b/radialog_amd/wcode.py
@@ -0,0 +1,74 @@
+import numpy as np
+
+CHUNK_K = 128
+CHUNK_BYTES = 64 * 52
+WINDOW = 15
+
+
+def pack_bf16(w_bits: np.ndarray) -> np.ndarray:
+    n, k = w_bits.shape
+    assert k % 32 == 0
+    nt = (n + 15) // 16
+    full = np.zeros((nt * 16, k), dtype=np.uint16)
+    full[:n] = w_bits
+    return np.ascontiguousarray(full.reshape(nt, 16, k // 32, 4, 8).transpose(0, 2, 3, 1, 4)).reshape(nt, k // 32, 64, 8)
+
+
+def encode(packed: np.ndarray):
+    nt, kc, lanes, eight = packed.shape
+    assert lanes == 64 and eight == 8 and kc % 4 == 0 and packed.dtype == np.uint16
+    kq = kc // 4
+    w = packed.astype(np.uint32)
+    h = (w >> 8) & 0x7F
+    lo = (w & 0xFF).astype(np.uint8)
+    sign = w >> 15
+    finite = h != 127
+    top = np.where(finite, h, 0).reshape(nt, -1).max(axis=1)
+    base = np.maximum(top.astype(np.int64) - WINDOW, 0)
+    idx = h.astype(np.int64) - base[:, None, None, None]
+    inside = (h == 0) | ((idx >= 1) & (idx <= WINDOW) & finite)
+    raw = ~inside.reshape(nt, -1).all(axis=1)
+    idx = np.where(inside & (h != 0), idx, 0).astype(np.uint32)
+
+    lo = lo.reshape(nt, kq, 4, 64, 8)
+    idx = idx.reshape(nt, kq, 4, 64, 8)
+    sign = sign.reshape(nt, kq, 4, 64, 8)
+    planes = np.zeros((nt, kq, CHUNK_BYTES), dtype=np.uint8)
+    lo_l = lo.transpose(0, 1, 3, 2, 4)
+    planes[:, :, 0:1024] = lo_l[:, :, :, 0:2, :].reshape(nt, kq, 1024)
+    planes[:, :, 1024:2048] = lo_l[:, :, :, 2:4, :].reshape(nt, kq, 1024)
+    e = np.arange(8)
+    nib = np.where(e < 4, 2 * e, 2 * (e - 4) + 1).astype(np.uint32)
+    ixw = (idx << (4 * nib)).sum(axis=-1, dtype=np.uint64).astype(np.uint32)
+    ixw = np.ascontiguousarray(ixw.transpose(0, 1, 3, 2)).astype("<u4")
+    planes[:, :, 2048:3072] = ixw.view(np.uint8).reshape(nt, kq, 1024)
+    j = np.arange(4)[:, None, None]
+    bit = ((2 * j + e // 4) + 8 * (e % 4)).astype(np.uint32)
+    sgw = (sign << bit).sum(axis=(2, 4), dtype=np.uint64).astype("<u4")
+    planes[:, :, 3072:3328] = np.ascontiguousarray(sgw).view(np.uint8).reshape(nt, kq, 256)
+    hdr = (base.astype(np.uint32) | (raw.astype(np.uint32) << 8)).astype(np.uint32)
+    return planes, hdr
+
+
+def decode(planes: np.ndarray, hdr: np.ndarray) -> np.ndarray:
+    nt, kq, nb = planes.shape
+    assert nb == CHUNK_BYTES
+    base = (hdr & 0xFF).astype(np.uint32)[:, None, None, None, None]
+    lo0 = planes[:, :, 0:1024].reshape(nt, kq, 64, 2, 8)
+    lo1 = planes[:, :, 1024:2048].reshape(nt, kq, 64, 2, 8)
+    lo = np.concatenate([lo0, lo1], axis=3).astype(np.uint32)
+    ixw = np.ascontiguousarray(planes[:, :, 2048:3072]).view("<u4").reshape(nt, kq, 64, 4, 1).astype(np.uint32)
+    sgw = np.ascontiguousarray(planes[:, :, 3072:3328]).view("<u4").reshape(nt, kq, 64, 1, 1).astype(np.uint32)
+    e = np.arange(8)
+    nib = np.where(e < 4, 2 * e, 2 * (e - 4) + 1).astype(np.uint32)
+    idx = (ixw >> (4 * nib)) & 0xF
+    j = np.arange(4)[:, None]
+    bit = ((2 * j + e // 4) + 8 * (e % 4)).astype(np.uint32)
+    sign = (sgw >> bit) & 1
+    h = np.where(idx != 0, base + idx, 0)
+    w = (sign << 15) | (h << 8) | lo
+    return np.ascontiguousarray(w.transpose(0, 1, 3, 2, 4)).reshape(nt, kq * 4, 64, 8).astype(np.uint16)
+
+
+def fallback_tiles(hdr: np.ndarray) -> int:
+    return int(((hdr >> 8) & 1).sum())
```
